# kristofbc/physical-interaction-video-prediction

Measured on AMD Instinct MI355X. Metric: predicted frames/sec (64x64x3, 10-step rollout), higher is better.
Workload: dtype f32; 1 GPU; CDNA rollout forward (Model.__call__, feed-self), batch 32/GPU, 10-frame 64x64x3 sequences, action-conditioned, num_masks=10, random-init weights; global_batch=32, parallelism=replicas x1

## Files before the change

### include/pivp_hip.h

```cpp
#ifndef PIVP_HIP_H
#define PIVP_HIP_H

#ifdef __cplusplus
extern "C" {
#endif

#define PIVP_OK 0
#define PIVP_ERR_BADARG (-1)
#define PIVP_ERR_LAUNCH (-2)
#define PIVP_ERR_STATE (-3)

#define PIVP_MODEL_CDNA 0
#define PIVP_MODEL_STP 1
#define PIVP_MODEL_DNA 2

#define PIVP_PRECISION_F32 0
#define PIVP_PRECISION_BF16 1
#define PIVP_PRECISION_BF16X3 2
#define PIVP_PRECISION_BF16X6 3
#define PIVP_PRECISION_FP16X3 4

int pivp_abi_version(void);

const char* pivp_build_digest(void);
const char* pivp_build_flags(void);

typedef struct pivp_plan pivp_plan_t;

typedef struct pivp_config {
    int batch;
    int seq_len;
    int height, width;
    int num_masks;
    int model_type;
    int use_state;
    int context_frames;
    int keep_activations;
    float ln_eps;
    int stp_zero_border;
    int action_dim;
    int state_dim;
} pivp_config_t;

int pivp_plan_create(const pivp_config_t* cfg, pivp_plan_t** out);
void pivp_plan_destroy(pivp_plan_t* plan);

int pivp_param_count(const pivp_plan_t* plan);
const char* pivp_param_name(const pivp_plan_t* plan, int idx);
long long pivp_param_numel(const pivp_plan_t* plan, int idx);
int pivp_plan_set_param(pivp_plan_t* plan, int idx, const float* dptr);

int pivp_plan_set_precision(pivp_plan_t* plan, int precision);
int pivp_plan_get_precision(const pivp_plan_t* plan);
int pivp_plan_set_deterministic(pivp_plan_t* plan, int on);
int pivp_plan_get_deterministic(const pivp_plan_t* plan);
enum { PIVP_OPT_SIDE_STREAM = 0, PIVP_OPT_FINISH_RIDER, PIVP_OPT_FUSE_ENC3, PIVP_OPT_LN_FOLD_TRAIN, PIVP_OPT_WGRAD_BATCH, PIVP_OPT_COUNT };
int pivp_plan_set_option(pivp_plan_t* plan, int option, int value);
int pivp_plan_get_option(const pivp_plan_t* plan, int option);
int pivp_plan_set_pack_cache(pivp_plan_t* plan, int on);
int pivp_plan_params_changed(pivp_plan_t* plan);

long long pivp_plan_workspace_bytes(const pivp_plan_t* plan);
int pivp_plan_set_workspace(pivp_plan_t* plan, void* dptr, long long bytes);

int pivp_reset_state(pivp_plan_t* plan, void* stream);

int pivp_rollout_forward(pivp_plan_t* plan, const float* images, const float* actions, const float* states,
                         const unsigned char* gt_select, float* gen_images, float* gen_states, float* results,
                         void* stream);

int pivp_rollout_predict(pivp_plan_t* plan, const float* context_images, const float* actions, const float* state0,
                         const float* track_in, int track_planes, int track_frame,
                         float* gen_images, float* gen_states, float* track_out, void* stream);

int pivp_plan_set_main_priority(pivp_plan_t* plan, int mode);

int pivp_plan_set_grad(pivp_plan_t* plan, int idx, float* dptr);
#define PIVP_GRAD_GROUPS 6
typedef void (*pivp_grad_group_cb)(void* user, int group);
int pivp_param_group(const pivp_plan_t* plan, int idx);
int pivp_param_group_by_name(const char* name);
int pivp_plan_set_grad_callback(pivp_plan_t* plan, pivp_grad_group_cb cb, void* user);
int pivp_plan_set_group_join(pivp_plan_t* plan, int join);
int pivp_plan_group_wait(pivp_plan_t* plan, int group, void* stream);
int pivp_rollout_backward(pivp_plan_t* plan, const float* images, const float* actions, const float* states,
                          const unsigned char* gt_select, const float* gen_images, const float* gen_states, void* stream);

int pivp_plan_set_profiling(pivp_plan_t* plan, int enable);
int pivp_plan_profile_read(pivp_plan_t* plan, double* ms_per_layer, int* launches_per_layer, double* flops_per_layer);

long long pivp_get_tap(pivp_plan_t* plan, const char* name, int step, float* out, void* stream);


int pivp_convlstm(const float* x, int cx, int ldx, const float* h_prev, int C, const float* w, const float* bias,
                  const float* c_in, float* c_out, float* h_out, int B, int H, int W, void* stream);

int pivp_convlstm_v(const float* x, int cx, int ldx, const float* h_prev, int C, const float* w, const float* bias,
                    const float* c_in, float* c_out, float* h_out, int B, int H, int W, int variant, void* stream);

long long pivp_convlstm_ln_scratch_floats(int B, int H, int W, int C);
int pivp_convlstm_ln(const float* x, int cx, int ldx, const float* h_prev, int C, const float* w, const float* bias,
                     const float* c_in, float* c_out, float* h_out, const float* gamma, const float* beta, float* ln_out,
                     int ldo, float* partials, float eps, int B, int H, int W, int variant, int* fused, void* stream);

long long pivp_lstm_bf16_weight_elems(int cin_total, int C);
int pivp_pack_lstm_bf16(const float* w, void* w_bf16, int cin_total, int C, void* stream);
int pivp_convlstm_bf16(const float* x, int cx, int ldx, const float* h_prev, int C, const void* w_bf16, const float* bias,
                       const float* c_in, float* c_out, float* h_out, float* gates_out, float* ln_part, int ln_cap,
                       int* ln_nparts, int B, int H, int W, int nch, void* stream);

int pivp_pack_lstm_bf16x3(const float* w, void* w_bf16, int cin_total, int C, void* stream);
int pivp_convlstm_bf16x3(const float* x, int cx, int ldx, const float* h_prev, int C, const void* w_bf16, const float* bias,
                         const float* c_in, float* c_out, float* h_out, float* gates_out, float* ln_part, int ln_cap,
                         int* ln_nparts, int B, int H, int W, int nch, void* stream);

int pivp_pack_lstm_bf16x6(const float* w, void* w_bf16, int cin_total, int C, void* stream);
int pivp_convlstm_bf16x6(const float* x, int cx, int ldx, const float* h_prev, int C, const void* w_bf16, const float* bias,
                         const float* c_in, float* c_out, float* h_out, float* gates_out, float* ln_part, int ln_cap,
                         int* ln_nparts, int B, int H, int W, int nch, void* stream);

int pivp_pack_lstm_fp16x3(const float* w, void* w_bf16, int cin_total, int C, int map_width, void* stream);
int pivp_convlstm_fp16x3(const float* x, int cx, int ldx, const float* h_prev, int C, const void* w_bf16, const float* bias,
                         const float* c_in, float* c_out, float* h_out, float* gates_out, float* ln_part, int ln_cap,
                         int* ln_nparts, int B, int H, int W, int nch, void* stream);

int pivp_deconv3x3s2_bf16(const float* x, int cin, int ldx, const float* w, const float* bias, float* out, int cout,
                          int ldo, int relu, int B, int Hin, int Win, void* stream);
int pivp_deconv3x3s2_bf16x3(const float* x, int cin, int ldx, const float* w, const float* bias, float* out, int cout,
                            int ldo, int relu, int B, int Hin, int Win, void* stream);
int pivp_deconv3x3s2_fp16x3(const float* x, int cin, int ldx, const float* w, const float* bias, float* out, int cout,
                            int ldo, int relu, int B, int Hin, int Win, float* scratch, void* stream);

long long pivp_conv5x5_bf16_weight_elems(int cin, int cout);
int pivp_conv5x5_bf16(const float* x, int cin, int ldx, const float* w, void* w_bf16, float* out, int cout, int ldo, int accum,
                      int B, int H, int W, void* stream);
int pivp_conv5x5_bf16x3(const float* x, int cin, int ldx, const float* w, void* w_bf16, float* out, int cout, int ldo, int accum,
                        int B, int H, int W, void* stream);
int pivp_conv5x5_bf16x6(const float* x, int cin, int ldx, const float* w, void* w_bf16, float* out, int cout, int ldo, int accum,
                        int B, int H, int W, void* stream);
int pivp_conv5x5_fp16x3(const float* x, int cin, int ldx, const float* w, void* w_bf16, float* out, int cout, int ldo, int accum,
                        int B, int H, int W, float* scratch, void* stream);
int pivp_conv5x5_ep(int precision, const float* x, int cin, int ldx, const float* w, void* w_bf16, float* out, int cout, int ldo, int accum,
                    const float* ep_src, int ep_ld, int ep_cols, int ep_mode, int no_split, float* scratch, int* applied,
                    int B, int H, int W, void* stream);
int pivp_conv5x5_ep_ksplit(int precision, int cin, int cout, int ldo, int accum, int no_split, int B, int H, int W);

int pivp_wgrad5x5_bf16(const float* x, int cx, int ldx, const float* h_prev, int C, const float* dG, float* dW, float* db,
                       int B, int H, int W, void* stream);
int pivp_wgrad5x5_bf16_batch(const float* x, int cx, int ldx, const float* h_prev, int C, const float* dG, float* dW, float* db,
                             int B, int H, int W, int tcount, long long ts_x, long long ts_h, long long ts_dG, void* stream);
int pivp_wgrad5x5_bf16_batch_form(const float* x, int cx, int ldx, const float* h_prev, int C, const float* dG, float* dW, float* db,
                                  int B, int H, int W, int tcount, long long ts_x, long long ts_h, long long ts_dG, int form, void* stream);
int pivp_wgrad5x5_bf16x6_batch(const float* x, int cx, int ldx, const float* h_prev, int C, const float* dG, float* dW, float* db,
                               int B, int H, int W, int tcount, long long ts_x, long long ts_h, long long ts_dG, void* stream);
int pivp_wgrad5x5_fp16x3_batch(const float* x, int cx, int ldx, const float* h_prev, int C, const float* dG, float* dW, float* db,
                               int B, int H, int W, int tcount, long long ts_x, long long ts_h, long long ts_dG, float* scratch, void* stream);

long long pivp_wgrad5x5_f32_part_floats(int cx, int C, int B, int H, int W, int form);
int pivp_wgrad5x5_f32_batch(const float* x, int cx, int ldx, const float* h_prev, int C, const float* dG, float* part, int overwrite,
                            float* dW, float* db, int B, int H, int W, int tcount, long long ts_x, long long ts_h, long long ts_dG, int form, void* stream);
int pivp_wgrad5x5_f32_reduce(int cx, int C, int has_h, float* part, float* dW, float* db, int B, int H, int W, int form, void* stream);
int pivp_wgrad5x5_f32_partition(int cx, int C, int has_h, int B, int H, int W, int form, int* geom8, int* segs, int seg_cap, int* nsegs,
                                int* slots, int slot_cap, int* nslots);
int pivp_conv5x5_f32(const float* x, int cin, int ldx, const float* wt, float* out, int cout, int B, int H, int W, void* stream);

int pivp_convlstm_train(const float* x, int cx, int ldx, const float* h_prev, int C, const float* w, const float* bias,
                        const float* c_in, float* c_out, float* h_out, float* gates_out, int B, int H, int W, void* stream);
int pivp_convlstm_backward(const float* x, int cx, int ldx, const float* h_prev, int C, const float* w, const float* gates,
                           const float* c_old, const float* c_new, const float* dh_a, int lda, const float* dh_b, int ldb,
                           float* dc, int dc_valid, float* dG, float* wt, float* d_in, float* dW, float* db,
                           int B, int H, int W, void* stream);
int pivp_conv_backward(int mode, const float* x, int cin, int ldx, const float* w, const float* dy, int cout, int ldy,
                       float* wt, float* dx, int lddx, int accum_dx, float* dW, float* db, int B, int Hin, int Win, void* stream);
long long pivp_conv_backward_part_floats(int mode, int cin, int cout, int B, int Hin, int Win);
int pivp_conv_wgrad_partial(int mode, const float* x, int cin, int ldx, const float* dy, int cout, int ldy, float* part,
                            float* dW, float* db, int B, int Hin, int Win, int repeats, void* stream);
int pivp_conv_wgrad_partial_batch(int mode, const float* x, int cin, int ldx, long long x_step_bytes, const float* dy, int cout, int ldy,
                                  long long dy_step_bytes, int tcount, int overwrite, float* part, float* dW, float* db, int B, int Hin, int Win,
                                  void* stream);
// ... 130 lines not shown
```

### physical-interaction-video-prediction_amd/csrc/igemm_f32.hip

```cpp
#include <stdlib.h>
#include <stdio.h>
#include <type_traits>

#include "lstm_gate_epilogue.h"

namespace pivp {

constexpr int IG_P = 36;

template <int WM, int NTB, int KG = 1>
constexpr int ig_lds_bytes() { return KG * 2 * (32 * WM + 32 * NTB) * IG_P * 4; }

#ifdef PIVP_F32_STAMPS
__device__ long long pivp_f32_stamps[2048 * 8];
#define F32_STAMP(i) do { if (threadIdx.x == 0 && blockIdx.x < 2048 && blockIdx.y == 0 && blockIdx.z == 0) { \
    pivp_f32_stamps[blockIdx.x * 4 + (i)] = (long long)wall_clock64(); pivp_f32_stamps[2048 * 4 + blockIdx.x * 4 + (i)] = (long long)clock64(); } } while (0)
#else
#define F32_STAMP(i)
#endif

template <int WM, int WN, int NTB, bool LSTM, int KG = 1>
__global__ __launch_bounds__(256 * KG, (KG == 1 && LSTM && WM < 4) ? 2 : 1) void igemm_f32_kernel(const IgemmDesc d) {
    F32_STAMP(0);
    PIVP_SET_MAIN_PRIO();
    static_assert(WM * WN == 4, "4 waves");
    static_assert(KG == 1 || (KG == 2 && LSTM), "the in-block K split serves the ConvLSTM tile only");
    static_assert(!LSTM || NTB == 4, "ConvLSTM blocks own 4 gates x 32 channels");
    constexpr int BM = 32 * WM;
    constexpr int BN = 32 * NTB;
    constexpr int CB = 8 * NTB;
    constexpr int CPW = LSTM ? CB / WN : 32 / WN;
    constexpr int GPT = 32 / CPW;
    constexpr int TPW = LSTM ? 4 / GPT : NTB / WN;
    extern __shared__ __attribute__((aligned(16))) float lds_all[];
    constexpr int A_FLOATS = BM * IG_P, B_FLOATS = BN * IG_P;
    const int gid = KG > 1 ? __builtin_amdgcn_readfirstlane((int)threadIdx.x >> 8) : 0;
    float* const lds = lds_all + gid * 2 * (A_FLOATS + B_FLOATS);

    const int tid = KG > 1 ? (int)threadIdx.x & 255 : (int)threadIdx.x;
    const int lane = tid & 63;
    const int wave = __builtin_amdgcn_readfirstlane(tid >> 6);
    const int wm = wave % WM, wn = wave / WM;
    const int phase = (int)gridDim.y - 1 - (int)blockIdx.y;
    const int n_nblk = LSTM ? (d.C / CB) : (d.N / BN);
    int lid = blockIdx.x;
    if ((gridDim.x & 7) == 0) lid = (blockIdx.x & 7) * (gridDim.x >> 3) + (blockIdx.x >> 3);
    const int n_mblk = d.n_mblk;
    const int nblk = pivp_fdiv(lid, d.fd_mb_mul, d.fd_mb_sh);
    const int mblk = lid - nblk * n_mblk;
    const int m0 = mblk * BM;
    const int cin = d.c0 + d.c1;
    const int ncc = cin >> 5;
    const int py = phase >> 1, px = phase & 1;
    const bool deconv = LSTM ? false : d.deconv != 0;
    const int ksz = LSTM ? 5 : d.ksize, pad = LSTM ? 2 : d.pad;
    const int nty_all = deconv ? 1 + py : ksz;
    const int ntx = deconv ? 1 + px : ksz;
    const int ksplit = LSTM ? 1 : (int)gridDim.z;
    const int nchunks_tot = nty_all * ntx * ncc;
    const int z_begin = ksplit > 1 ? (int)((unsigned)(nchunks_tot * (int)blockIdx.z) / (unsigned)ksplit) : 0;
    const int z_end = ksplit > 1 ? (int)((unsigned)(nchunks_tot * ((int)blockIdx.z + 1)) / (unsigned)ksplit) : nchunks_tot;
    const int nchunks_all = z_end - z_begin;
    const int nchunks = nchunks_all / KG;
    const int chunk0 = z_begin + gid * nchunks;
    const int HWg = d.Hg * d.Wg;

    constexpr int NA = (BM * 8 + 255) / 256;
    constexpr int NB = BN * 8 / 256;
    constexpr unsigned OOB = 0xC0000000u;
    const int cvec = tid & 7;
    const int prow = tid >> 3;
    const __amdgpu_buffer_rsrc_t rs0 = __builtin_amdgcn_make_buffer_rsrc(const_cast<float*>(d.x0), 0, d.bytes0, 0x00020000);
    const __amdgpu_buffer_rsrc_t rs1 = __builtin_amdgcn_make_buffer_rsrc(const_cast<float*>(d.c1 ? d.x1 : d.x0), 0, d.c1 ? d.bytes1 : d.bytes0, 0x00020000);
    const __amdgpu_buffer_rsrc_t rsw = __builtin_amdgcn_make_buffer_rsrc(const_cast<float*>(d.w), 0, d.bytesw, 0x00020000);
    int a_off0[NA], a_off1[NA];
    unsigned a_mask[NA];
    auto anchors = [&]() {
#pragma unroll
    for (int j = 0; j < NA; ++j) {
        const int m = m0 + prow + 32 * j;
        if (m < d.M && prow + 32 * j < BM) {
            const int b = pivp_fdiv(m, d.fd_hw_mul, d.fd_hw_sh);
            const int rem = m - b * HWg;
            const int ay = pivp_fdiv(rem, d.fd_w_mul, d.fd_w_sh);
            const int ax = rem - ay * d.Wg;
            const int iy0 = ay * d.in_step, ix0 = ax * d.in_step;
            const int pix = b * d.Hin * d.Win + iy0 * d.Win + ix0;
            a_off0[j] = (pix * d.ld0 + cvec * 4) * 4;
            a_off1[j] = (pix * d.ld1 + cvec * 4) * 4;
            unsigned colm = 0, m25 = 0;
            if (deconv) {
#pragma unroll
                for (int t = 0; t < 5; ++t) {
                    const int dxx = (px + 1 - (px ? 2 * t : 1)) >> 1;
                    if (t < ntx && (unsigned)(ix0 + dxx) < (unsigned)d.Win) colm |= 1u << t;
                }
#pragma unroll
                for (int t = 0; t < 5; ++t) {
                    const int dyy = (py + 1 - (py ? 2 * t : 1)) >> 1;
                    if (t < nty_all && (unsigned)(iy0 + dyy) < (unsigned)d.Hin) m25 |= colm << (5 * t);
                }
            } else {
                auto run = [](int lo, int hi) -> unsigned { return hi >= lo ? ((2u << hi) - 1u) & ~((1u << lo) - 1u) : 0u; };
                colm = run(max(pad - ix0, 0), min(d.Win - 1 + pad - ix0, ntx - 1));
                const int rlo = max(pad - iy0, 0), rhi = min(d.Hin - 1 + pad - iy0, nty_all - 1);
                const unsigned rows = rhi >= rlo ? 0x108421u & ((2u << (5 * rhi)) - 1u) & ~((1u << (5 * rlo)) - 1u) : 0u;
                m25 = colm * rows;
            }
            a_mask[j] = m25;
        } else {
            a_off0[j] = a_off1[j] = 0;
            a_mask[j] = 0;
        }
    }
    };
    int b_goff[NB];
#pragma unroll
    for (int j = 0; j < NB; ++j) {
        const int r = prow + 32 * j;
        const int col = LSTM ? (r / CB) * d.C + nblk * CB + (r % CB) : nblk * BN + r;
        b_goff[j] = (col * 32 + cvec * 4) * 4;
    }
    const int lds_wa = (prow * IG_P + cvec * 4);

    f32x4 ras[2][NA];
    f32x4 rbs[2][NB];

    int l_cc = 0, l_ty = 0, l_tx = 0;
    if (KG > 1 || ksplit > 1) {
        const int tap = pivp_fdiv(chunk0, d.fd_cc_mul, d.fd_cc_sh);
        l_cc = chunk0 - tap * ncc; l_ty = LSTM ? tap / 5 : tap / ntx; l_tx = tap - l_ty * ntx;
    }
    int s_delta = 0, s_ld = 0, s_wbase = 0;
    unsigned s_bit = 0;
    bool s_first = true;
    int t_dy = 0, t_dx = 0, t_wi = 0, t_cbase = 0;
    auto stage_a = [&]() {
        if (deconv) {
            const int ky = py ? 2 * l_ty : 1, kx = px ? 2 * l_tx : 1;
            t_dy = (py + 1 - ky) >> 1; t_dx = (px + 1 - kx) >> 1; t_wi = ky * 3 + kx;
        } else {
            t_dy = l_ty - pad; t_dx = l_tx - pad; t_wi = l_ty * ksz + l_tx;
        }
        s_bit = __builtin_amdgcn_readfirstlane(1u << (l_ty * 5 + l_tx));
        const int ch = l_cc << 5;
        s_first = ch < d.c0;
        s_ld = s_first ? d.ld0 : d.ld1;
        t_cbase = s_first ? ch : ch - d.c0;
    };
    auto stage_b = [&]() {
        s_delta = __builtin_amdgcn_readfirstlane(((t_dy * d.Win + t_dx) * s_ld + t_cbase) * 4);
    };
    auto stage_c = [&]() {
        s_wbase = __builtin_amdgcn_readfirstlane((t_wi * (d.wcin >> 5) + l_cc) * (d.wN ? d.wN : d.N) * 128);
        ++l_cc;
        const bool w0 = l_cc == ncc;
        l_cc = w0 ? 0 : l_cc;
        l_tx += w0 ? 1 : 0;
        const bool w1 = l_tx == ntx;
        l_tx = w1 ? 0 : l_tx;
        l_ty += w1 ? 1 : 0;
    };
    auto stage_begin = [&]() { stage_a(); stage_b(); stage_c(); };
    auto load_piece = [&](auto SET, auto J) {
        constexpr int j = decltype(J)::value;
        f32x4 (&ra)[NA] = ras[decltype(SET)::value];
        f32x4 (&rb)[NB] = rbs[decltype(SET)::value];
        if constexpr (j < NA) {
            const bool ok = (a_mask[j] & s_bit) != 0;
            unsigned off = ok ? (unsigned)((s_first ? a_off0[j] : a_off1[j]) + s_delta) : OOB;
            ra[j] = __builtin_bit_cast(f32x4, s_first ? __builtin_amdgcn_raw_buffer_load_b128(rs0, off, 0, 0)
                                                      : __builtin_amdgcn_raw_buffer_load_b128(rs1, off, 0, 0));
        } else if constexpr (j < NA + NB) {
            rb[j - NA] = __builtin_bit_cast(f32x4, __builtin_amdgcn_raw_buffer_load_b128(rsw, b_goff[j - NA], s_wbase, 0));
        }
    };
    auto store_piece = [&](auto SET, auto J, int buf) {
        constexpr int j = decltype(J)::value;
        const f32x4 (&ra)[NA] = ras[decltype(SET)::value];
        const f32x4 (&rb)[NB] = rbs[decltype(SET)::value];
        if constexpr (j < NA) {
            if (BM >= 32 * (j + 1)) *reinterpret_cast<f32x4*>(lds + buf * A_FLOATS + lds_wa + 32 * j * IG_P) = ra[j];
        } else if constexpr (j < NA + NB) {
            *reinterpret_cast<f32x4*>(lds + 2 * A_FLOATS + buf * B_FLOATS + lds_wa + 32 * (j - NA) * IG_P) = rb[j - NA];
        }
    };

    constexpr int NACC = LSTM ? (TPW == 1 ? 4 : TPW == 2 ? 2 : 1) : 1;
    f32x16 accs[NACC][TPW];
    f32x16 (&acc)[TPW] = accs[0];

    const int half = lane >> 5;
    const int l31 = lane & 31;
    const int a_off = (wm * 32 + l31) * IG_P + 4 * half;
    int b_off[TPW];
#pragma unroll
    for (int t = 0; t < TPW; ++t) {
        int row;
        if (LSTM) row = (t * GPT + l31 / CPW) * CB + wn * CPW + (l31 % CPW);
        else      row = (wn * TPW + t) * 32 + l31;
        b_off[t] = 2 * A_FLOATS + row * IG_P + 4 * half;
    }

    constexpr int NST = NA + NB;
    static_assert(NST <= 8, "staging pieces must fit the 16 micro-steps twice");
    constexpr int PRE = NST < 8 ? NST : 0;
    f32x4 fa[2];
    f32x4 fb[2][TPW];
    auto read_frag0 = [&](int slot) {
        fa[0] = *reinterpret_cast<const f32x4*>(lds + slot * A_FLOATS + a_off);
#pragma unroll
        for (int t = 0; t < TPW; ++t) fb[0][t] = *reinterpret_cast<const f32x4*>(lds + slot * B_FLOATS + b_off[t]);
    };
    auto chunk = [&](auto LOAD, auto STORE, auto SET, auto PAR, int buf) {
        constexpr bool do_load = decltype(LOAD)::value;
        constexpr bool do_store = decltype(STORE)::value;
        using OTHER = std::integral_constant<int, decltype(SET)::value ^ 1>;
        const float* As = lds + buf * A_FLOATS + a_off;
        const float* Bs = lds + buf * B_FLOATS;
        read_frag0(buf);
        __builtin_amdgcn_sched_barrier(0);
        auto micro = [&](auto Q, auto S2) {
            constexpr int q = decltype(Q)::value, s2 = decltype(S2)::value, step = q * 4 + s2;
            constexpr int cur = q & 1, nxt = cur ^ 1;
            constexpr int ci = NACC == 1 ? 0 : NACC == 2 ? decltype(PAR)::value : 2 * decltype(PAR)::value + (q & 1);
            if constexpr (s2 == 0 && q < 3) {
                fa[nxt] = *reinterpret_cast<const f32x4*>(As + 8 * (q + 1));
#pragma unroll
                for (int t = 0; t < TPW; ++t) fb[nxt][t] = *reinterpret_cast<const f32x4*>(Bs + b_off[t] + 8 * (q + 1));
            }
#pragma unroll
            for (int t = 0; t < TPW; ++t)
                accs[ci][t] = __builtin_amdgcn_mfma_f32_32x32x2f32(fa[cur][s2], fb[cur][t][s2], accs[ci][t], 0, 0, 0);
            if constexpr (do_load && PRE == 0 && step == 0) stage_begin();
            if constexpr (do_load && PRE > 0 && step == PRE) stage_a();
            if constexpr (do_load && PRE > 0 && step == PRE + 1) stage_b();
            if constexpr (do_load && PRE > 0 && step == PRE + 2) stage_c();
            if constexpr (do_load && step < NST) load_piece(SET, std::integral_constant<int, step>{});
            if constexpr (do_store && step >= 16 - NST) store_piece(OTHER{}, std::integral_constant<int, step - (16 - NST)>{}, buf ^ 1);
            __builtin_amdgcn_sched_barrier(0);
        };
        auto qgroup = [&](auto Q) {
            micro(Q, std::integral_constant<int, 0>{}); micro(Q, std::integral_constant<int, 1>{});
            micro(Q, std::integral_constant<int, 2>{}); micro(Q, std::integral_constant<int, 3>{});
        };
        qgroup(std::integral_constant<int, 0>{}); qgroup(std::integral_constant<int, 1>{});
        qgroup(std::integral_constant<int, 2>{}); qgroup(std::integral_constant<int, 3>{});
    };
    using S0 = std::integral_constant<int, 0>; using S1 = std::integral_constant<int, 1>;
    auto load_all = [&](auto SET) {
        load_piece(SET, std::integral_constant<int, 0>{}); load_piece(SET, std::integral_constant<int, 1>{});
        load_piece(SET, std::integral_constant<int, 2>{}); load_piece(SET, std::integral_constant<int, 3>{});
        load_piece(SET, std::integral_constant<int, 4>{}); load_piece(SET, std::integral_constant<int, 5>{});
        load_piece(SET, std::integral_constant<int, 6>{}); load_piece(SET, std::integral_constant<int, 7>{});
    };
    auto store_all = [&](auto SET, int buf) {
        store_piece(SET, std::integral_constant<int, 0>{}, buf); store_piece(SET, std::integral_constant<int, 1>{}, buf);
        store_piece(SET, std::integral_constant<int, 2>{}, buf); store_piece(SET, std::integral_constant<int, 3>{}, buf);
        store_piece(SET, std::integral_constant<int, 4>{}, buf); store_piece(SET, std::integral_constant<int, 5>{}, buf);
        store_piece(SET, std::integral_constant<int, 6>{}, buf); store_piece(SET, std::integral_constant<int, 7>{}, buf);
    };
    auto sync = [&]() { __syncthreads(); };
    auto load_b = [&](auto SET) {
        if constexpr (NB > 0) load_piece(SET, std::integral_constant<int, NA + 0>{});
        if constexpr (NB > 1) load_piece(SET, std::integral_constant<int, NA + 1>{});
        if constexpr (NB > 2) load_piece(SET, std::integral_constant<int, NA + 2>{});
        if constexpr (NB > 3) load_piece(SET, std::integral_constant<int, NA + 3>{});
    };
    auto load_a = [&](auto SET) {
        if constexpr (NA > 0) load_piece(SET, std::integral_constant<int, 0>{});
        if constexpr (NA > 1) load_piece(SET, std::integral_constant<int, 1>{});
        if constexpr (NA > 2) load_piece(SET, std::integral_constant<int, 2>{});
        if constexpr (NA > 3) load_piece(SET, std::integral_constant<int, 3>{});
    };
    static_assert(NA <= 4 && NB <= 4, "load_a / load_b unroll four pieces each");

    if (nchunks > 0) { stage_begin(); load_b(S0{}); }
    __builtin_amdgcn_sched_barrier(0);
    anchors();
    if (nchunks > 0) load_a(S0{});
    __builtin_amdgcn_sched_barrier(0);

    constexpr int OWNR = LSTM ? 16 / GPT : 1;
    float cpre[OWNR];
    float bj = 0.f, bi = 0.f, bf = 0.f, bo = 0.f;
    if constexpr (LSTM) {
        const int C = d.C, ch = nblk * CB + wn * CPW + (l31 % CPW), grp = l31 / CPW;
        bj = d.bias[ch]; bi = d.bias[C + ch]; bf = d.bias[2 * C + ch] + 1.0f; bo = d.bias[3 * C + ch];
        const __amdgpu_buffer_rsrc_t rsci = __builtin_amdgcn_make_buffer_rsrc(const_cast<float*>(d.cstate_in), 0, d.M * C * 4, 0x00020000);
        const int voc = ((m0 + wm * 32 + 4 * half + (GPT > 1 ? grp : 0)) * C + ch) * 4;
#pragma unroll
        for (int k = 0; k < OWNR; ++k) {
            const int srow = GPT == 1 ? (k & 3) + 8 * (k >> 2) : GPT == 2 ? 2 * (k & 1) + 8 * (k >> 1) : 8 * k;
            cpre[k] = __builtin_bit_cast(float, __builtin_amdgcn_raw_buffer_load_b32(rsci, voc, srow * C * 4, 0));
        }
    }

#pragma unroll
    for (int a = 0; a < NACC; ++a)
#pragma unroll
        for (int n = 0; n < TPW; ++n)
#pragma unroll
            for (int r = 0; r < 16; ++r) accs[a][n][r] = 0.f;
    if (nchunks > 0) {
        store_all(S0{}, 0);
        if (nchunks > 1) { stage_begin(); load_all(S1{}); }
        if constexpr (PRE > 0) stage_begin();
        __syncthreads();
        F32_STAMP(1);
        int it = 0;
        for (; it + 3 < nchunks; it += 2) {
            chunk(std::true_type{}, std::true_type{}, S0{}, S0{}, 0); sync();
            chunk(std::true_type{}, std::true_type{}, S1{}, S1{}, 1); sync();
        }
        const int rest = nchunks - it;
        if (rest == 3) {
            chunk(std::true_type{}, std::true_type{}, S0{}, S0{}, 0); sync();
            chunk(std::false_type{}, std::true_type{}, S1{}, S1{}, 1); sync();
            chunk(std::false_type{}, std::false_type{}, S0{}, S0{}, 0);
        } else if (rest == 2) {
            chunk(std::false_type{}, std::true_type{}, S0{}, S0{}, 0); sync();
            chunk(std::false_type{}, std::false_type{}, S0{}, S1{}, 1);
        } else {
            chunk(std::false_type{}, std::false_type{}, S0{}, S0{}, 0);
        }
    }
    F32_STAMP(2);
    if constexpr (NACC > 1) {
#pragma unroll
        for (int t = 0; t < TPW; ++t)
#pragma unroll
            for (int r = 0; r < 16; ++r) {
                if constexpr (NACC == 2) accs[0][t][r] = accs[0][t][r] + accs[1][t][r];
                else accs[0][t][r] = (accs[0][t][r] + accs[1][t][r]) + (accs[2][t][r] + accs[3][t][r]);
            }
    }

    if constexpr (KG > 1) {
        __syncthreads();
        float* xch = lds_all;
        if (gid == 1) {
#pragma unroll
            for (int t = 0; t < TPW; ++t)
#pragma unroll
                for (int r = 0; r < 16; ++r) xch[(t * 16 + r) * 256 + tid] = accs[0][t][r];
        }
        __syncthreads();
        if (gid == 1) {
            if (LSTM && d.ln_part) { __syncthreads(); __syncthreads(); __syncthreads(); }
            return;
        }
#pragma unroll
        for (int t = 0; t < TPW; ++t)
#pragma unroll
            for (int r = 0; r < 16; ++r) accs[0][t][r] += xch[(t * 16 + r) * 256 + tid];
    }

    auto tile_stats = [&](const float* v, auto ownmask, auto NV, int b, int slot) {
        constexpr int nv = decltype(NV)::value;
        float s1 = 0.f, c1 = 0.f;
#pragma unroll
        for (int i = 0; i < nv; ++i)
            if ((ownmask >> i) & 1) { s1 += v[i]; c1 += 1.f; }
        s1 = wave_sum(s1); c1 = wave_sum(c1);
        __syncthreads();
        if (lane == 0) { lds[wave] = s1; lds[4 + wave] = c1; }
        __syncthreads();
        const float cnt = (lds[4] + lds[5]) + (lds[6] + lds[7]);
        const float mean = ((lds[0] + lds[1]) + (lds[2] + lds[3])) / cnt;
        float q = 0.f;
#pragma unroll
        for (int i = 0; i < nv; ++i)
            if ((ownmask >> i) & 1) { const float dd = v[i] - mean; q = fmaf(dd, dd, q); }
        q = wave_sum(q);
        if (lane == 0) lds[8 + wave] = q;
        __syncthreads();
        if (tid == 0) {
            float* p = d.ln_part + ((size_t)b * d.ln_nparts + slot) * 4;
            p[0] = cnt; p[1] = mean; p[2] = (lds[8] + lds[9]) + (lds[10] + lds[11]); p[3] = 0.f;
        }
    };
    if constexpr (LSTM) {
        const int C = d.C;
        const int ch = nblk * CB + wn * CPW + (l31 % CPW);
        const int grp = l31 / CPW;
        const int M = d.M;
        const __amdgpu_buffer_rsrc_t rsc = __builtin_amdgcn_make_buffer_rsrc(d.cstate_out, 0, M * C * 4, 0x00020000);
        const __amdgpu_buffer_rsrc_t rsh = __builtin_amdgcn_make_buffer_rsrc(d.hout, 0, M * C * 4, 0x00020000);
        const __amdgpu_buffer_rsrc_t rsg = __builtin_amdgcn_make_buffer_rsrc(d.gates_out ? d.gates_out : d.hout, 0, d.gates_out ? M * C * 16 : 0, 0x00020000);
        const int mlane = m0 + wm * 32 + 4 * half + (GPT > 1 ? grp : 0);
        const int vo = (mlane * C + ch) * 4, vog = (mlane * 4 * C + ch) * 4;
        float sv[OWNR];
        unsigned own = 0;
#pragma unroll
        for (int k = 0; k < OWNR; ++k) {
            float g4[4];
#pragma unroll
            for (int t = 0; t < 4 / GPT; ++t) {
                float rows[GPT], got[GPT];
#pragma unroll
                for (int g = 0; g < GPT; ++g) rows[g] = acc[t][k * GPT + g];
                gate_exchange<GPT, CPW>(rows, grp, got);
#pragma unroll
                for (int g = 0; g < GPT; ++g) g4[t * GPT + g] = got[g];
            }
            const int srow = GPT == 1 ? (k & 3) + 8 * (k >> 2) : GPT == 2 ? 2 * (k & 1) + 8 * (k >> 1) : 8 * k;
            const int so = srow * C * 4;
            const LstmCell cell = lstm_cell<GateActF32>(g4, bj, bi, bf, bo, cpre[k]);
            __builtin_amdgcn_raw_buffer_store_b32(__builtin_bit_cast(unsigned, cell.c), rsc, vo, so, 0);
            __builtin_amdgcn_raw_buffer_store_b32(__builtin_bit_cast(unsigned, cell.h), rsh, vo, so, 0);
            const bool in = mlane + srow < M;
            sv[k] = in ? cell.h : 0.f;
            own |= in ? 1u << k : 0u;
            if (d.gates_out) {
                const int sog = so * 4;
                __builtin_amdgcn_raw_buffer_store_b32(__builtin_bit_cast(unsigned, cell.aj), rsg, vog, sog, 0);
                __builtin_amdgcn_raw_buffer_store_b32(__builtin_bit_cast(unsigned, cell.ai), rsg, vog, sog + C * 4, 0);
                __builtin_amdgcn_raw_buffer_store_b32(__builtin_bit_cast(unsigned, cell.af), rsg, vog, sog + C * 8, 0);
                __builtin_amdgcn_raw_buffer_store_b32(__builtin_bit_cast(unsigned, cell.ao), rsg, vog, sog + C * 12, 0);
            }
        }
        if (d.ln_part) {
            const int b = pivp_fdiv(m0, d.fd_hw_mul, d.fd_hw_sh);
            tile_stats(sv, own, std::integral_constant<int, OWNR>{}, b, ((m0 - b * HWg) / BM) * n_nblk + nblk);
        }
    } else if (!deconv && d.out_step == 1 && d.Hout == d.Hg && d.Wout == d.Wg && !d.bias && !d.relu && !d.accum && !d.ln_part &&
               (long long)d.M * d.ldo * 4 < (1LL << 31)) {
        const __amdgpu_buffer_rsrc_t rso = __builtin_amdgcn_make_buffer_rsrc(d.out, 0, d.M * d.ldo * 4, 0x00020000);
        const int vo = ((m0 + wm * 32 + 4 * half) * d.ldo + nblk * BN + wn * TPW * 32 + l31) * 4;
        const int row4 = __builtin_amdgcn_readfirstlane(d.ldo * 4);
        if (ksplit > 1) {
            if (nchunks > 0) {
#pragma unroll
                for (int r = 0; r < 16; ++r)
#pragma unroll
                    for (int t = 0; t < TPW; ++t)
                        __builtin_amdgcn_raw_ptr_buffer_atomic_fadd_f32(acc[t][r], rso, vo + t * 128, ((r & 3) + 8 * (r >> 2)) * row4, 0);
            }
        } else {
#pragma unroll
            for (int r = 0; r < 16; ++r)
#pragma unroll
                for (int t = 0; t < TPW; ++t) {
                    const float v = acc[t][r];
                    __builtin_amdgcn_raw_buffer_store_b32(__builtin_bit_cast(unsigned, v), rso, vo + t * 128, ((r & 3) + 8 * (r >> 2)) * row4, 0);
                }
        }
    } else {
        const int oy0 = deconv ? py : 0, ox0 = deconv ? px : 0;
        float sv[16 * TPW];
        unsigned long long own = 0;
#pragma unroll
        for (int r = 0; r < 16; ++r) {
            const int m = m0 + wm * 32 + (r & 3) + 8 * (r >> 2) + 4 * half;
            if (m < d.M) {
                const int b = pivp_fdiv(m, d.fd_hw_mul, d.fd_hw_sh);
                const int rem = m - b * HWg;
                const int ay = pivp_fdiv(rem, d.fd_w_mul, d.fd_w_sh);
                const int ax = rem - ay * d.Wg;
                const int opix = (ay * d.out_step + oy0) * d.Wout + ax * d.out_step + ox0;
                const size_t o = ((size_t)b * d.Hout * d.Wout + opix) * d.ldo;
#pragma unroll
                for (int t = 0; t < TPW; ++t) {
                    const int col = nblk * BN + (wn * TPW + t) * 32 + l31;
                    if (ksplit > 1) {
                        if (nchunks > 0) atomicAdd(d.out + o + col, acc[t][r]);
                    } else {
                        float v = acc[t][r] + (d.bias ? d.bias[col] : 0.f);
                        if (d.relu) v = fmaxf(v, 0.f);
                        if (d.accum) v += d.out[o + col];
                        d.out[o + col] = v;
                        sv[t * 16 + r] = v; own |= 1ull << (t * 16 + r);
                    }
                }
            }
        }
        if (d.ln_part) {
            const int b = pivp_fdiv(m0, d.fd_hw_mul, d.fd_hw_sh);
            tile_stats(sv, own, std::integral_constant<int, 16 * TPW>{}, b,
                       (((m0 - b * HWg) / BM) * n_nblk + nblk) * (int)gridDim.y + phase);
        }
    }
#ifdef PIVP_F32_STAMPS
    asm volatile("s_waitcnt vmcnt(0)" ::: "memory");
    F32_STAMP(3);
#endif
}

template <int WM, int WN, int NTB, bool LSTM, int KG = 1>
static int launch_igemm(const IgemmDesc& d, hipStream_t stream, int ksplit = 1, int* ln_nparts = nullptr) {
    constexpr int BM = 32 * WM, BN = 32 * NTB;
    const int n_nblk = LSTM ? (d.C / (8 * NTB)) : (d.N / BN);
    const int mblk = (d.M + BM - 1) / BM;
    constexpr int lds_bytes = ig_lds_bytes<WM, NTB, KG>();
    static PerDeviceOnce once;
    if (pivp_ensure_dyn_lds(once, reinterpret_cast<const void*>(&igemm_f32_kernel<WM, WN, NTB, LSTM, KG>), lds_bytes) != PIVP_OK) return PIVP_ERR_LAUNCH;
    dim3 grid(mblk * n_nblk, d.nphase, ksplit);
    IgemmDesc dd = d;
    dd.n_mblk = mblk;
    pivp_fastdiv((unsigned)mblk, &dd.fd_mb_mul, &dd.fd_mb_sh);
    pivp_fastdiv((unsigned)(d.Hg * d.Wg), &dd.fd_hw_mul, &dd.fd_hw_sh);
    pivp_fastdiv((unsigned)d.Wg, &dd.fd_w_mul, &dd.fd_w_sh);
    pivp_fastdiv((unsigned)((d.c0 + d.c1) >> 5), &dd.fd_cc_mul, &dd.fd_cc_sh);
    const int hwg = d.Hg * d.Wg;
    const int np = (hwg / BM) * n_nblk * d.nphase;
    dd.ln_nparts = (d.ln_part && ksplit == 1 && hwg % BM == 0 && np <= d.ln_cap) ? np : 0;
    if (!dd.ln_nparts) dd.ln_part = nullptr;
    if (ln_nparts) *ln_nparts = dd.ln_nparts;
    hipLaunchKernelGGL((igemm_f32_kernel<WM, WN, NTB, LSTM, KG>), grid, dim3(256 * KG), lds_bytes, stream, dd);
    return PIVP_LAUNCH_STATUS();
}

int igemm_validate(const IgemmDesc& d, bool lstm) {
    PIVP_CHECK_ARG(d.x0 && d.w && d.c0 > 0 && d.c0 % 32 == 0 && d.c1 % 32 == 0 && d.c1 >= 0);
    PIVP_CHECK_ARG(d.c1 == 0 || d.x1);
    PIVP_CHECK_ARG(d.ld0 >= d.c0 && d.ld0 % 4 == 0 && (d.c1 == 0 || (d.ld1 >= d.c1 && d.ld1 % 4 == 0)));
    PIVP_CHECK_ARG(d.B > 0 && d.Hin > 0 && d.Win > 0 && d.Hg > 0 && d.Wg > 0 && d.in_step >= 1);
    PIVP_CHECK_ARG(d.M == d.B * d.Hg * d.Wg);
    PIVP_CHECK_ARG(d.deconv ? (d.nphase == 4 && d.in_step == 1 && d.out_step == 2) : (d.nphase == 1 && d.ksize >= 1 && d.ksize <= 5 && d.pad >= 0));
    PIVP_CHECK_ARG(d.bytes0 > 0 && d.bytesw > 0 && (d.c1 == 0 || d.bytes1 > 0));
    PIVP_CHECK_ARG(d.wcin >= d.c0 + d.c1 && d.wcin % 32 == 0);
    if (lstm) {
        PIVP_CHECK_ARG(d.C > 0 && d.C % 32 == 0 && d.N == 4 * d.C && d.bias && d.cstate_in && d.cstate_out && d.hout);
        PIVP_CHECK_ARG(d.nphase == 1 && d.in_step == 1 && d.Hg == d.Hin && d.Wg == d.Win && d.ksize == 5 && d.pad == 2 && !d.deconv);
        PIVP_CHECK_ARG((long long)d.M * d.C * 4 < (1LL << 31));
    } else {
        PIVP_CHECK_ARG(d.out && d.N % 32 == 0 && d.N >= 32 && d.ldo >= d.N);
        PIVP_CHECK_ARG(d.out_step >= 1 && d.Hout > 0 && d.Wout > 0);
        PIVP_CHECK_ARG((d.Hg - 1) * d.out_step + (d.deconv ? 1 : 0) < d.Hout && (d.Wg - 1) * d.out_step + (d.deconv ? 1 : 0) < d.Wout);
    }
    return PIVP_OK;
}

int igemm_lstm(const IgemmDesc& d, hipStream_t stream, int variant, int* ln_nparts) {
    int rc = igemm_validate(d, true);
    if (rc != PIVP_OK) return rc;
    if (variant == 0) {
        const long nb = d.C / 32;
        if ((long)(d.M / 64) * nb >= 512) variant = 2;
        else if ((long)(d.M / 64) * nb >= 256) variant = 4;
        else variant = 3;
    }
    switch (variant) {
        case 4:
            if (((25 * ((d.c0 + d.c1) >> 5)) & 1) == 0) return launch_igemm<2, 2, 4, true, 2>(d, stream, 1, ln_nparts);
            return launch_igemm<2, 2, 4, true>(d, stream, 1, ln_nparts);
        case 1: return launch_igemm<4, 1, 4, true>(d, stream, 1, ln_nparts);
        case 2: return launch_igemm<2, 2, 4, true>(d, stream, 1, ln_nparts);
        case 3: {
            const int ncc = (d.c0 + d.c1) >> 5;
            if (((25 * ncc) & 1) == 0) return launch_igemm<1, 4, 4, true, 2>(d, stream, 1, ln_nparts);
            return launch_igemm<1, 4, 4, true>(d, stream, 1, ln_nparts);
        }
    }
    return PIVP_ERR_BADARG;
}

static bool dgrad_choice(const IgemmDesc& d, int& bt, int& bks) {
    if (!((d.ksplit_ok || d.no_ksplit) && !d.deconv && !d.bias && !d.relu && !d.accum && d.ksize * d.ksize * ((d.c0 + d.c1) / 32) > 40)) return false;
    const int ks_max = d.no_ksplit ? 1 : 10;
    const int nt = d.N / 32;
    struct Tile { int wm, wn, ntb; double eff; int resident; };
    static const Tile tiles[] = {{2, 2, 2, 0.80, 4}, {4, 1, 1, 0.70, 3}, {4, 1, 2, 0.90, 2}, {4, 1, 3, 0.95, 2}, {4, 1, 4, 1.00, 1}, {2, 2, 4, 0.95, 2}, {1, 4, 4, 0.80, 3}};
    static const double fixed_taps[] = {3.0, 1.5, 1.0, 1.0};
    static const double alone[] = {0.90, 1.0, 1.0, 1.0};
    const int cus = pivp_cu_count();
    bt = -1; bks = 1;
    double bcost = 1e300;
    const int nchunks = d.ksize * d.ksize * ((d.c0 + d.c1) / 32);
    const double split_penalty = 1.01 + 0.14 * (d.M >= 32768 ? 1.0 : d.M / 32768.0);
    for (int t = 0; t < 7; ++t) {
        if (nt % tiles[t].ntb) continue;
        const int bm = 32 * tiles[t].wm, bn = 32 * tiles[t].ntb;
        const long mb = (d.M + bm - 1) / bm, nb = d.N / bn;
        for (int ks = 1; ks <= ks_max && ks * 8 <= nchunks; ++ks) {
            const long blocks = mb * nb * ks;
            const long per_cu = (blocks + cus - 1) / cus;
            const int res = (int)(per_cu < tiles[t].resident ? per_cu : tiles[t].resident);
            const double taps = (double)(d.ksize * d.ksize) / ks;
            const double cost = (double)per_cu * bm * bn * (taps + fixed_taps[res - 1]) / (tiles[t].eff * alone[res - 1]) * (ks > 1 ? split_penalty : 1.0);
            if (cost < bcost) { bcost = cost; bt = t; bks = ks; }
        }
    }
    return bt >= 0;
}
int igemm_conv_ksplit(const IgemmDesc& d) {
    int bt, bks;
    return dgrad_choice(d, bt, bks) ? bks : 1;
}

int igemm_conv(const IgemmDesc& d, hipStream_t stream, int* ln_nparts) {
    int rc = igemm_validate(d, false);
    if (rc != PIVP_OK) return rc;
    int bt = -1, bks = 1;
    const bool dgrad = dgrad_choice(d, bt, bks);
    const bool aligned = d.ldo % 4 == 0 && ((uintptr_t)d.out & 15) == 0 && (!d.bias || ((uintptr_t)d.bias & 15) == 0);
    const bool tile_ok = deconv_tile_ok(d);
    switch (conv_form(d.deconv, d.c0 + d.c1, d.N, d.B, tile_ok ? d.Hin : 1, d.Win, aligned, dgrad, d.ksize, d.M)) {
        case ConvForm::DeconvTile: return deconv_tile(d, stream, ln_nparts);
        case ConvForm::LongKDgrad:
            switch (bt) {
                case 0: return launch_igemm<2, 2, 2, false>(d, stream, bks, ln_nparts);
                case 1: return launch_igemm<4, 1, 1, false>(d, stream, bks, ln_nparts);
                case 2: return launch_igemm<4, 1, 2, false>(d, stream, bks, ln_nparts);
                case 3: return launch_igemm<4, 1, 3, false>(d, stream, bks, ln_nparts);
                case 4: return launch_igemm<4, 1, 4, false>(d, stream, bks, ln_nparts);
                case 5: return launch_igemm<2, 2, 4, false>(d, stream, bks, ln_nparts);
                case 6: return launch_igemm<1, 4, 4, false>(d, stream, bks, ln_nparts);
            }
            return PIVP_ERR_BADARG;
        case ConvForm::Small1: case ConvForm::Small2: case ConvForm::Small3: return igemm_small(d, stream, ln_nparts);
        case ConvForm::F32_128x32: return launch_igemm<4, 1, 1, false>(d, stream, 1, ln_nparts);
        case ConvForm::F32_128x64: return launch_igemm<4, 1, 2, false>(d, stream, 1, ln_nparts);
        case ConvForm::F32_128x96: return launch_igemm<4, 1, 3, false>(d, stream, 1, ln_nparts);
        case ConvForm::F32_128x128: return launch_igemm<4, 1, 4, false>(d, stream, 1, ln_nparts);
        case ConvForm::F32_64x64: return launch_igemm<2, 2, 2, false>(d, stream, 1, ln_nparts);
        case ConvForm::F32_64x128: return launch_igemm<2, 2, 4, false>(d, stream, 1, ln_nparts);
        case ConvForm::F32_32x128: return launch_igemm<1, 4, 4, false>(d, stream, 1, ln_nparts);
    }
    return PIVP_ERR_BADARG;
}

}

#ifdef PIVP_F32_STAMPS
extern "C" int pivp_debug_f32_stamps(long long* out, int n) {
    return hipMemcpyFromSymbol(out, HIP_SYMBOL(pivp::pivp_f32_stamps), sizeof(long long) * n) == hipSuccess ? 0 : -2;
}
#endif

PIVP_DEFINE_MAIN_PRIO_SETTER(igemm_f32)
// ... 1 lines not shown
```

### physical-interaction-video-prediction_amd/csrc/pivp_c_api.hip

```cpp
#include <string.h>
#include <string>
#include <vector>

#include "../../include/pivp_hip.h"
#include "../../include/pivp_data.h"
#include "../../include/pivp_conv_forms.h"
#include "pivp_host.h"

using namespace pivp;

namespace pivp {

long long view_bytes(int B, int H, int W, int ld) { return (long long)B * H * W * ld * 4; }
bool fits31(long long v) { return v > 0 && v < (1LL << 31); }
int run_convlstm(const float* x, int cx, int ldx, const float* h_prev, int C, const float* w, const float* bias,
                 const float* c_in, float* c_out, float* h_out, int B, int H, int W, hipStream_t s, const ConvLstmOpts& o) {
    const LnIn* const ln_in = o.ln_in;
    const bool l2d = operand_l2_direct(o.operand);
    if ((o.w_bf16 != nullptr) != (o.operand != Operand::F32)) return PIVP_ERR_BADARG;
    IgemmDesc d;
    memset(&d, 0, sizeof(d));
    if (ln_in) {
        if (!convlstm_ln_in_ok(o.operand, cx, ldx, C, B, H, W) || !ln_in->gamma || !ln_in->beta || !ln_in->part || ln_in->np <= 0 || ln_in->part == o.ln_out.part)
            return PIVP_ERR_BADARG;
        d.in_g = ln_in->gamma; d.in_b = ln_in->beta; d.in_part = ln_in->part; d.in_np = ln_in->np; d.in_eps = ln_in->eps;
    }
    d.x0 = x; d.c0 = cx; d.ld0 = ldx; d.x1 = h_prev; d.c1 = h_prev ? C : 0; d.ld1 = C; d.wcin = cx + C;
    d.w = w; d.bias = bias;
    d.B = B; d.Hin = H; d.Win = W; d.Hg = H; d.Wg = W; d.in_step = 1;
    d.N = 4 * C; d.M = B * H * W;
    d.nphase = 1; d.deconv = 0; d.ksize = 5; d.pad = 2;
    const long long b0 = view_bytes(B, H, W, ldx), b1 = view_bytes(B, H, W, C), bw = 25LL * (cx + C) * 4 * C * 4;
    if (!fits31(b0) || !fits31(b1) || !fits31(bw) || (o.gates_out && !fits31(4 * b1))) return PIVP_ERR_BADARG;
    d.bytes0 = (int)b0; d.bytes1 = (int)b1; d.bytesw = (int)bw;
    d.out_step = 1; d.Hout = H; d.Wout = W;
    d.cstate_in = c_in; d.cstate_out = c_out; d.hout = h_out; d.C = C; d.gates_out = o.gates_out;
    d.ln_part = o.ln_out.part; d.ln_cap = o.ln_out.cap;
    if (l2d && !convlstm_bf16_ok(d)) return w ? igemm_lstm(d, s, 0, o.ln_out.nparts) : PIVP_ERR_BADARG;
    if (o.w_bf16) return convlstm_bf16(d, o.w_bf16, s, o.operand, o.ln_out.nparts, (l2d && o.variant != 16 && o.variant != 32) ? 0 : o.variant);
    return igemm_lstm(d, s, o.variant, o.ln_out.nparts);
}

bool convlstm_ln_in_ok(Operand form, int cx, int ldx, int C, int B, int H, int W) {
    return operand_l2_direct(form) && cx <= 64 && ldx == cx && cx % 8 == 0 && C % 16 == 0 && H % 8 == 0 && W % 16 == 0;
}
static int conv3x3s2_desc(IgemmDesc& d, const float* x, int cin, int ldx, const float* w, const float* bias, float* out, int cout,
                          int ldo, int relu, int B, int Hin, int Win, int accum) {
    if (Hin % 2 || Win % 2) return PIVP_ERR_BADARG;
    memset(&d, 0, sizeof(d));
    d.x0 = x; d.c0 = cin; d.ld0 = ldx; d.wcin = cin; d.w = w; d.bias = bias;
    d.B = B; d.Hin = Hin; d.Win = Win; d.Hg = Hin / 2; d.Wg = Win / 2; d.in_step = 2;
    d.N = cout; d.M = B * d.Hg * d.Wg;
    d.nphase = 1; d.deconv = 0; d.ksize = 3; d.pad = 1;
    const long long b0 = view_bytes(B, Hin, Win, ldx), bw = 9LL * cin * cout * 4;
    if (!fits31(b0) || !fits31(bw)) return PIVP_ERR_BADARG;
    d.bytes0 = (int)b0; d.bytesw = (int)bw;
    d.out_step = 1; d.Hout = d.Hg; d.Wout = d.Wg; d.out = out; d.ldo = ldo; d.relu = relu; d.accum = accum;
    return PIVP_OK;
}
int run_conv3x3s2(const float* x, int cin, int ldx, const float* w, const float* bias, float* out, int cout,
                  int ldo, int relu, int B, int Hin, int Win, hipStream_t s, int accum) {
    IgemmDesc d;
    int rc = conv3x3s2_desc(d, x, cin, ldx, w, bias, out, cout, ldo, relu, B, Hin, Win, accum);
    if (rc != PIVP_OK) return rc;
    return igemm_conv(d, s);
}

static void conv3x3s2_ln_desc(IgemmDesc& d, const float* x_raw, int cin, const float* w, const float* bias, float* out, int cout, int ldo,
                              int relu, int B, int Hin, int Win) {
    memset(&d, 0, sizeof(d));
    d.x0 = x_raw; d.c0 = cin; d.ld0 = cin; d.wcin = cin; d.w = w; d.bias = bias;
    d.B = B; d.Hin = Hin; d.Win = Win; d.Hg = Hin / 2; d.Wg = Win / 2; d.in_step = 2;
    d.N = cout; d.M = B * d.Hg * d.Wg;
    d.nphase = 1; d.deconv = 0; d.ksize = 3; d.pad = 1;
    d.out_step = 1; d.Hout = d.Hg; d.Wout = d.Wg; d.out = out; d.ldo = ldo; d.relu = relu;
}
bool conv3x3s2_ln_ok(int cin, int cout, int B, int Hin, int Win) {
    if (Hin % 2 || Win % 2 || cin % 32 || cout % 32) return false;
    IgemmDesc d;
    conv3x3s2_ln_desc(d, nullptr, cin, nullptr, nullptr, nullptr, cout, cout, 0, B, Hin, Win);
    return igemm_in_ln_ok(d) && fits31(view_bytes(B, Hin, Win, cin)) && fits31(9LL * cin * cout * 4);
}
int run_conv3x3s2_ln(const float* x_raw, int cin, const float* w, const float* bias, float* out, int cout, int ldo, int relu,
                     int B, int Hin, int Win, hipStream_t s, const LnIn& ln, const Conv3x3LnOpts& o) {
    if (!x_raw || !w || !out || !ln.gamma || !ln.beta || !ln.part || ln.np <= 0 || !conv3x3s2_ln_ok(cin, cout, B, Hin, Win)) return PIVP_ERR_BADARG;
    IgemmDesc d;
    conv3x3s2_ln_desc(d, x_raw, cin, w, bias, out, cout, ldo, relu, B, Hin, Win);
    d.bytes0 = (int)view_bytes(B, Hin, Win, cin); d.bytesw = (int)(9LL * cin * cout * 4);
    d.in_g = ln.gamma; d.in_b = ln.beta; d.in_part = ln.part; d.in_np = ln.np; d.in_eps = ln.eps;
    d.in_out = o.keep.out; d.in_out_ld = o.keep.ld; d.in_stat_out = o.keep.stat;
    if (o.fuse3 && o.fuse3->e3) {
        if (cout != 64 || ldo != 64 || !relu || !bias) return PIVP_ERR_BADARG;
        d.f3_w = o.fuse3->w3; d.f3_b = o.fuse3->b3; d.f3_action = o.fuse3->action; d.f3_state = o.fuse3->state; d.f3_wcs = o.fuse3->wcs; d.f3_bcs = o.fuse3->bcs;
        d.f3_out = o.fuse3->e3; d.f3_state_out = o.fuse3->state_out; d.f3_use_state = o.fuse3->use_state;
    }
    int rc = igemm_validate(d, false);
    if (rc != PIVP_OK) return rc;
    return igemm_small(d, s);
}

static int deconv3x3s2_desc(IgemmDesc& d, const float* x0, int c0, int ld0, const float* x1, int c1, int ld1, const float* w, const float* bias,
                            float* out, int cout, int ldo, int relu, int B, int Hin, int Win) {
    memset(&d, 0, sizeof(d));
    d.x0 = x0; d.c0 = c0; d.ld0 = ld0; d.x1 = x1; d.c1 = x1 ? c1 : 0; d.ld1 = ld1; d.wcin = c0 + d.c1; d.w = w; d.bias = bias;
    d.B = B; d.Hin = Hin; d.Win = Win; d.Hg = Hin; d.Wg = Win; d.in_step = 1;
    d.N = cout; d.M = B * Hin * Win;
    d.nphase = 4; d.deconv = 1; d.ksize = 3; d.pad = 1;
    const long long b0 = view_bytes(B, Hin, Win, ld0), b1 = d.c1 ? view_bytes(B, Hin, Win, ld1) : 0, bw = 9LL * d.wcin * cout * 4;
    if (!fits31(b0) || (d.c1 && !fits31(b1)) || !fits31(bw)) return PIVP_ERR_BADARG;
    d.bytes0 = (int)b0; d.bytes1 = (int)b1; d.bytesw = (int)bw;
    d.out_step = 2; d.Hout = 2 * Hin; d.Wout = 2 * Win; d.out = out; d.ldo = ldo; d.relu = relu;
    return PIVP_OK;
}
static bool deconv_form_ok(Operand form, const float* wscale_part) { return form != Operand::BF16X6 && (!operand_needs_scale(form) || wscale_part); }
int run_deconv3x3s2(const float* x, int cin, int ldx, const float* w, const float* bias, float* out, int cout,
                    int ldo, int relu, int B, int Hin, int Win, hipStream_t s, const DeconvOpts& o) {
    if (!deconv_form_ok(o.operand, o.wscale_part)) return PIVP_ERR_BADARG;
    IgemmDesc d;
    int rc = deconv3x3s2_desc(d, x, cin, ldx, nullptr, 0, 0, w, bias, out, cout, ldo, relu, B, Hin, Win);
// ... 222 lines not shown
    if (rc != PIVP_OK) return rc;
    return fork_end(a.fork);
}

int run_layernorm(const float* x, const float* g, const float* b, float* out, float* partials, int B, int n, int C,
                  int ldo, float eps, int relu, hipStream_t s, const LayerNormOpts& o) {
    if (o.fused_nparts <= 0) {
        int rc = ln_stats(x, partials, B, n, s);
        if (rc != PIVP_OK) return rc;
    }
    return ln_apply(x, partials, g, b, out, B, n, C, ldo, eps, relu, s, o.stat_out, o.fused_nparts);
}

__global__ __launch_bounds__(256) void select_frames_kernel(const float* __restrict__ gt, const float* __restrict__ gen,
                                                            const unsigned char* __restrict__ take, float* __restrict__ out,
                                                            int frame_numel) {
    const int b = blockIdx.y;
    const float* src = take[b] ? gt : gen;
    const size_t base = (size_t)b * frame_numel;
    for (int i = (blockIdx.x * 256 + threadIdx.x) * 4; i < frame_numel; i += gridDim.x * 1024)
        *reinterpret_cast<f32x4*>(out + base + i) = *reinterpret_cast<const f32x4*>(src + base + i);
}

int run_select_frames(const float* gt, const float* gen, const unsigned char* take, float* out, int B, int frame_numel, hipStream_t s) {
    if (!gt || !gen || !take || !out || B <= 0 || frame_numel <= 0 || frame_numel % 4) return PIVP_ERR_BADARG;
    hipLaunchKernelGGL(select_frames_kernel, dim3(8, B), dim3(256), 0, s, gt, gen, take, out, frame_numel);
    return PIVP_LAUNCH_STATUS();
}

int run_conv_backward(const ConvBwdArgs& a, hipStream_t s) {
    const int mode = a.mode, B = a.B, Hin = a.Hin, Win = a.Win;
    const int Hout = mode ? 2 * Hin : Hin / 2, Wout = mode ? 2 * Win : Win / 2;
    int rc = PIVP_OK;
    if (a.y) { rc = relu_mask(a.dy, a.ldy, a.y, a.ldyy, a.cout, (long)B * Hout * Wout, s, a.dy_add, a.ld_add); if (rc != PIVP_OK) return rc; }
    else if (a.dy_add) { rc = add_strided(a.dy, a.ldy, a.dy_add, a.ld_add, a.cout, (long)B * Hout * Wout, s); if (rc != PIVP_OK) return rc; }
    hipStream_t sw;
    rc = fork_begin(a.fork, s, &sw);
    if (rc != PIVP_OK) return rc;
    if (a.dx) {
        if (!a.wt_ready) {
            rc = repack_transpose(a.w, a.wt, 9, a.cin, a.cout, 0, s);
            if (rc != PIVP_OK) return rc;
        }
        DeconvOpts o{};
        o.accum = a.accum_dx; o.operand = a.operand;
        rc = mode ? run_conv3x3s2(a.dy, a.cout, a.ldy, a.wt, nullptr, a.dx, a.cin, a.lddx, 0, B, Hout, Wout, s, a.accum_dx)
                  : run_deconv3x3s2(a.dy, a.cout, a.ldy, a.wt, nullptr, a.dx, a.cin, a.lddx, 0, B, Hout, Wout, s, o);
        if (rc != PIVP_OK) return rc;
    }
    if (!a.dW) return PIVP_OK;
    WgradDesc d;
    conv3x3s2_wgrad_geom(d, mode, a.cin, a.cout, B, Hin, Win);
    d.x0 = a.x; d.ld0 = a.ldx; d.dy = a.dy; d.ldy = a.ldy; d.dw = a.dW; d.db = a.db; d.part = a.part;
    rc = run_wgrad(d, sw, Operand::F32);
    if (rc != PIVP_OK) return rc;
    return fork_end(a.fork);
}

}

#ifndef PIVP_BUILD_DIGEST
#define PIVP_BUILD_DIGEST "unstamped"
#endif
extern "C" const char* pivp_build_digest(void) { return PIVP_BUILD_DIGEST; }
#ifndef PIVP_BUILD_FLAGS
#define PIVP_BUILD_FLAGS ""
#endif
extern "C" const char* pivp_build_flags(void) { return PIVP_BUILD_FLAGS; }
extern "C" int pivp_abi_version(void) { return 17; }

static bool ep_args_ok(const float* ep_src, int ep_ld, int ep_cols, int ep_mode, int cout) {
    if (ep_mode < 0 || ep_mode > 2) return false;
    if (!ep_src || !ep_mode) return true;
    return ep_ld >= (ep_cols < cout ? ep_cols : cout);
}
static bool form_serves_map(Operand form, int B, int H, int W) { return form == Operand::F32 || packed_tiles_serve(H, W, B); }
extern "C" int pivp_convlstm(const float* x, int cx, int ldx, const float* h_prev, int C, const float* w, const float* bias,
                             const float* c_in, float* c_out, float* h_out, int B, int H, int W, void* stream) {
    if (!x || !w || !bias || !c_in || !c_out || !h_out) return PIVP_ERR_BADARG;
    return run_convlstm(x, cx, ldx, h_prev, C, w, bias, c_in, c_out, h_out, B, H, W, (hipStream_t)stream);
}
extern "C" int pivp_convlstm_v(const float* x, int cx, int ldx, const float* h_prev, int C, const float* w, const float* bias,
                               const float* c_in, float* c_out, float* h_out, int B, int H, int W, int variant, void* stream) {
    if (!x || !w || !bias || !c_in || !c_out || !h_out || variant < 0 || variant > 4) return PIVP_ERR_BADARG;
    ConvLstmOpts o{};
    o.variant = variant;
    return run_convlstm(x, cx, ldx, h_prev, C, w, bias, c_in, c_out, h_out, B, H, W, (hipStream_t)stream, o);
}
extern "C" int pivp_convlstm_train(const float* x, int cx, int ldx, const float* h_prev, int C, const float* w, const float* bias,
                                   const float* c_in, float* c_out, float* h_out, float* gates_out, int B, int H, int W, void* stream) {
    if (!x || !w || !bias || !c_in || !c_out || !h_out || !gates_out) return PIVP_ERR_BADARG;
    ConvLstmOpts o{};
    o.gates_out = gates_out;
    return run_convlstm(x, cx, ldx, h_prev, C, w, bias, c_in, c_out, h_out, B, H, W, (hipStream_t)stream, o);
}
static int convlstm_backward_op(const float* x, int cx, int ldx, const float* h_prev, int C, const float* w, const float* gates,
                                const float* c_old, const float* c_new, const float* dh_a, int lda, const float* dh_b, int ldb,
                                float* dc, int dc_valid, float* dG, float* wt, float* d_in, float* dW, float* db,
                                int B, int H, int W, void* stream, int dx_only) {
    if (!x || !w || !gates || !c_old || !c_new || !dc || !dG || !wt || !d_in || !dW || !db) return PIVP_ERR_BADARG;
    ConvLstmBwdArgs a{};
    a.x = x; a.cx = cx; a.ldx = ldx; a.h_prev = h_prev; a.C = C; a.w = w; a.gates = gates; a.c_old = c_old; a.c_new = c_new;
    a.dh_a = dh_a; a.lda = lda; a.dh_b = dh_b; a.ldb = ldb; a.dc = dc; a.dc_valid = dc_valid; a.dG = dG; a.wt = wt; a.d_in = d_in;
    a.dW = dW; a.db = db; a.B = B; a.H = H; a.W = W;
    a.dx_only = dx_only;
    return run_convlstm_backward(a, (hipStream_t)stream);
}
extern "C" int pivp_convlstm_backward(const float* x, int cx, int ldx, const float* h_prev, int C, const float* w, const float* gates,
                                      const float* c_old, const float* c_new, const float* dh_a, int lda, const float* dh_b, int ldb,
                                      float* dc, int dc_valid, float* dG, float* wt, float* d_in, float* dW, float* db,
                                      int B, int H, int W, void* stream) {
    return convlstm_backward_op(x, cx, ldx, h_prev, C, w, gates, c_old, c_new, dh_a, lda, dh_b, ldb, dc, dc_valid, dG, wt, d_in, dW, db, B, H, W, stream, 0);
}
extern "C" int pivp_conv_backward(int mode, const float* x, int cin, int ldx, const float* w, const float* dy, int cout, int ldy,
                                  float* wt, float* dx, int lddx, int accum_dx, float* dW, float* db, int B, int Hin, int Win,
                                  void* stream) {
    if (!x || !w || !dy || !wt || !dW || !db || mode < 0 || mode > 1) return PIVP_ERR_BADARG;
    ConvBwdArgs a{};
    a.mode = mode; a.x = x; a.cin = cin; a.ldx = ldx; a.w = w; a.dy = const_cast<float*>(dy); a.cout = cout; a.ldy = ldy;
    a.wt = wt; a.dx = dx; a.lddx = lddx; a.accum_dx = accum_dx; a.dW = dW; a.db = db; a.B = B; a.Hin = Hin; a.Win = Win;
    return run_conv_backward(a, (hipStream_t)stream);
}
extern "C" long long pivp_conv_backward_part_floats(int mode, int cin, int cout, int B, int Hin, int Win) {
    if (mode < 0 || mode > 1 || cin <= 0 || cout <= 0 || B <= 0 || Hin <= 0 || Win <= 0) return PIVP_ERR_BADARG;
    return conv_backward_part_floats(mode, cin, cout, B, Hin, Win);
}
extern "C" int pivp_conv_wgrad_partial(int mode, const float* x, int cin, int ldx, const float* dy, int cout, int ldy, float* part,
                                       float* dW, float* db, int B, int Hin, int Win, int repeats, void* stream) {
    if (!x || !dy || !part || !dW || !db || mode < 0 || mode > 1 || repeats < 1) return PIVP_ERR_BADARG;
    WgradDesc desc;
    conv3x3s2_wgrad_geom(desc, mode, cin, cout, B, Hin, Win);
    desc.x0 = x; desc.ld0 = ldx; desc.dy = dy; desc.ldy = ldy; desc.dw = dW; desc.db = db; desc.part = part;
    for (int r = 0; r < repeats; ++r) {
        const int rc = run_wgrad(desc, (hipStream_t)stream, Operand::F32);
        if (rc != PIVP_OK) return rc;
    }
    return igemm_wgrad_reduce(desc, (hipStream_t)stream);
}
extern "C" int pivp_conv_wgrad_partial_batch(int mode, const float* x, int cin, int ldx, long long x_step_bytes, const float* dy, int cout, int ldy,
                                             long long dy_step_bytes, int tcount, int overwrite, float* part, float* dW, float* db, int B, int Hin, int Win,
                                             void* stream) {
    if (!x || !dy || !part || !dW || !db || mode < 0 || mode > 1 || tcount < 1) return PIVP_ERR_BADARG;
    WgradDesc d;
    conv3x3s2_wgrad_geom(d, mode, cin, cout, B, Hin, Win);
    d.x0 = x; d.ld0 = ldx; d.dy = dy; d.ldy = ldy; d.dw = dW; d.db = db;
    d.tcount = tcount; d.ts_x0 = x_step_bytes; d.ts_dy = dy_step_bytes;
    d.part = part; d.part_overwrite = overwrite ? 1 : 0;
    return run_wgrad(d, (hipStream_t)stream, Operand::F32);
}
extern "C" int pivp_conv_wgrad_partial_reduce(int mode, int cin, int cout, float* part, float* dW, float* db, int B, int Hin, int Win, void* stream) {
    if (!part || !dW || !db || mode < 0 || mode > 1) return PIVP_ERR_BADARG;
    WgradDesc d;
    conv3x3s2_wgrad_geom(d, mode, cin, cout, B, Hin, Win);
    d.part = part; d.dw = dW; d.db = db;
    return igemm_wgrad_reduce(d, (hipStream_t)stream);
}
static void lstm_wgrad_op(WgradDesc& d, const float* x, int cx, int ldx, const float* h_prev, int C, const float* dG, float* dW, float* db,
                          int B, int H, int W, int tcount, long long ts_x, long long ts_h, long long ts_dG) {
    lstm_wgrad_geom(d, cx, C, B, H, W);
    d.x0 = x; d.ld0 = ldx; d.x1 = h_prev; d.dy = dG; d.dw = dW; d.db = db;
    d.tcount = tcount; d.ts_x0 = ts_x; d.ts_x1 = ts_h; d.ts_dy = ts_dG;
}
extern "C" long long pivp_wgrad5x5_f32_part_floats(int cx, int C, int B, int H, int W, int form) {
    if (cx <= 0 || C <= 0 || B <= 0 || H <= 0 || W <= 0 || form < 0 || form > 2) return PIVP_ERR_BADARG;
    return lstm_wgrad_part_floats(cx, C, B, H, W, form, 0);
}
extern "C" int pivp_wgrad5x5_f32_batch(const float* x, int cx, int ldx, const float* h_prev, int C, const float* dG, float* part, int overwrite,
                                       float* dW, float* db, int B, int H, int W, int tcount, long long ts_x, long long ts_h, long long ts_dG, int form,
                                       void* stream) {
// ... 160 lines not shown
    o.operand = Operand::FP16X3; o.ascale_part = scratch;
    return run_conv5x5_bf16(x, cin, ldx, (const unsigned short*)w_bf16, out, cout, ldo, accum, B, H, W, (hipStream_t)stream, o);
}
extern "C" int pivp_conv5x5_ep(int precision, const float* x, int cin, int ldx, const float* w, void* w_bf16, float* out, int cout, int ldo, int accum,
                               const float* ep_src, int ep_ld, int ep_cols, int ep_mode, int no_split, float* scratch, int* applied,
                               int B, int H, int W, void* stream) {
    if (applied) *applied = 0;
    if (precision < 1 || precision > 4 || !x || !w || !w_bf16 || !out || cin <= 0 || cout <= 0 || B <= 0 || H <= 0 || W <= 0) return PIVP_ERR_BADARG;
    const Operand form = (Operand)precision;
    if (!form_serves_map(form, B, H, W) || (operand_needs_scale(form) && (!scratch || ldx != cin)) || !ep_args_ok(ep_src, ep_ld, ep_cols, ep_mode, cout))
        return PIVP_ERR_BADARG;
    int rc = pack_lstm_bf16(w, (unsigned short*)w_bf16, cin, cout, (hipStream_t)stream, form, conv5x5_bf16_rows(cout), operand_l2_direct(form) ? 1 : 0);
    if (rc != PIVP_OK) return rc;
    if (operand_needs_scale(form)) {
        rc = absmax_partials(x, (long)B * H * W * cin, scratch, (hipStream_t)stream);
        if (rc != PIVP_OK) return rc;
    }
    const EpSpec ep{ep_src, ep_ld, ep_cols, ep_mode, applied};
    Conv5x5Bf16Opts o{};
    o.operand = form; o.no_split = no_split ? 1 : 0;
    if (operand_needs_scale(form)) o.ascale_part = scratch;
    if (ep_src && ep_mode) o.ep = &ep;
    return run_conv5x5_bf16(x, cin, ldx, (const unsigned short*)w_bf16, out, cout, ldo, accum, B, H, W, (hipStream_t)stream, o);
}
extern "C" int pivp_conv5x5_ep_ksplit(int precision, int cin, int cout, int ldo, int accum, int no_split, int B, int H, int W) {
    if (precision < 1 || precision > 4 || cin <= 0 || cout <= 0 || ldo < cout || B <= 0 || H <= 0 || W <= 0) return PIVP_ERR_BADARG;
    IgemmDesc d;
    static float dummy;
    if (conv5x5_bf16_desc(d, &dummy, cin, cin, &dummy, cout, ldo, accum, B, H, W) != PIVP_OK) return PIVP_ERR_BADARG;
    if (no_split) d.ksplit_ok = 0;
    return conv5x5_bf16_ksplit(d, (Operand)precision);
}
static int lstm_wgrad_packed_op(Operand operand, const float* x, int cx, int ldx, const float* h_prev, int C, const float* dG, float* dW, float* db, int B, int H,
                                int W, int tcount, long long ts_x, long long ts_h, long long ts_dG, int form, const float* dy_absmax, void* stream) {
    WgradDesc d;
    lstm_wgrad_op(d, x, cx, ldx, h_prev, C, dG, dW, db, B, H, W, tcount, ts_x, ts_h, ts_dG);
    d.form = form;
    if (dy_absmax) { d.dy_absmax = dy_absmax; d.dy_absmax_stride = 72; }
    return run_wgrad(d, (hipStream_t)stream, operand);
}
extern "C" int pivp_wgrad5x5_bf16(const float* x, int cx, int ldx, const float* h_prev, int C, const float* dG, float* dW, float* db,
                                  int B, int H, int W, void* stream) {
    if (!x || !dG || !dW || C <= 0 || cx <= 0) return PIVP_ERR_BADARG;
    return lstm_wgrad_packed_op(Operand::BF16, x, cx, ldx, h_prev, C, dG, dW, db, B, H, W, 1, 0, 0, 0, 0, nullptr, stream);
}
extern "C" int pivp_wgrad5x5_fp16x3_batch(const float* x, int cx, int ldx, const float* h_prev, int C, const float* dG, float* dW, float* db,
                                          int B, int H, int W, int tcount, long long ts_x, long long ts_h, long long ts_dG, float* scratch, void* stream) {
    if (!x || !dG || !dW || !scratch || C <= 0 || cx <= 0 || tcount < 1 || B <= 0 || H <= 0 || W <= 0) return PIVP_ERR_BADARG;
    if (!form_serves_map(Operand::FP16X3, B, H, W)) return PIVP_ERR_BADARG;
    for (int j = 0; j < tcount; ++j) {
        const int rc = absmax_partials(reinterpret_cast<const float*>(reinterpret_cast<const char*>(dG) + j * ts_dG), (long)B * H * W * 4 * C,
                                       scratch + (size_t)j * 72, (hipStream_t)stream);
        if (rc != PIVP_OK) return rc;
    }
    return lstm_wgrad_packed_op(Operand::FP16X3, x, cx, ldx, h_prev, C, dG, dW, db, B, H, W, tcount, ts_x, ts_h, ts_dG, 0, scratch, stream);
}
extern "C" int pivp_wgrad5x5_bf16x6_batch(const float* x, int cx, int ldx, const float* h_prev, int C, const float* dG, float* dW, float* db,
                                          int B, int H, int W, int tcount, long long ts_x, long long ts_h, long long ts_dG, void* stream) {
    if (!x || !dG || !dW || C <= 0 || cx <= 0 || tcount < 1) return PIVP_ERR_BADARG;
    return lstm_wgrad_packed_op(Operand::BF16X6, x, cx, ldx, h_prev, C, dG, dW, db, B, H, W, tcount, ts_x, ts_h, ts_dG, 0, nullptr, stream);
}
extern "C" int pivp_wgrad5x5_bf16_batch(const float* x, int cx, int ldx, const float* h_prev, int C, const float* dG, float* dW, float* db,
                                        int B, int H, int W, int tcount, long long ts_x, long long ts_h, long long ts_dG, void* stream) {
    if (!x || !dG || !dW || C <= 0 || cx <= 0 || tcount < 1) return PIVP_ERR_BADARG;
    return lstm_wgrad_packed_op(Operand::BF16, x, cx, ldx, h_prev, C, dG, dW, db, B, H, W, tcount, ts_x, ts_h, ts_dG, 0, nullptr, stream);
}
extern "C" int pivp_wgrad5x5_bf16_batch_form(const float* x, int cx, int ldx, const float* h_prev, int C, const float* dG, float* dW, float* db,
                                             int B, int H, int W, int tcount, long long ts_x, long long ts_h, long long ts_dG, int form, void* stream) {
    if (!x || !dG || !dW || C <= 0 || cx <= 0 || tcount < 1 || form < 0 || form > 2) return PIVP_ERR_BADARG;
    return lstm_wgrad_packed_op(Operand::BF16, x, cx, ldx, h_prev, C, dG, dW, db, B, H, W, tcount, ts_x, ts_h, ts_dG, form, nullptr, stream);
}
static int convlstm_ln_cap(int H, int W, int C) {
    const int tiles = ((H * W + 31) / 32) * (C / 32), slices = ln_stats_slices(H * W * C);
    return tiles > slices ? tiles : slices;
}
extern "C" long long pivp_convlstm_ln_scratch_floats(int B, int H, int W, int C) {
    if (B <= 0 || H <= 0 || W <= 0 || C <= 0 || C % 32) return PIVP_ERR_BADARG;
    return (long long)B * convlstm_ln_cap(H, W, C) * 4;
}
extern "C" int pivp_convlstm_ln(const float* x, int cx, int ldx, const float* h_prev, int C, const float* w, const float* bias,
                                const float* c_in, float* c_out, float* h_out, const float* gamma, const float* beta,
                                float* ln_out, int ldo, float* partials, float eps, int B, int H, int W, int variant, int* fused,
                                void* stream) {
    if (!x || !w || !bias || !c_in || !c_out || !h_out || !gamma || !beta || !ln_out || !partials || variant < 0 || variant > 4)
        return PIVP_ERR_BADARG;
    if (C <= 0 || C % 32) return PIVP_ERR_BADARG;
    int np = 0;
    ConvLstmOpts o{};
    o.variant = variant; o.ln_out.part = partials; o.ln_out.cap = convlstm_ln_cap(H, W, C); o.ln_out.nparts = &np;
    int rc = run_convlstm(x, cx, ldx, h_prev, C, w, bias, c_in, c_out, h_out, B, H, W, (hipStream_t)stream, o);
    if (rc != PIVP_OK) return rc;
    if (fused) *fused = np > 0;
    LayerNormOpts lo{};
    lo.fused_nparts = np;
    return run_layernorm(h_out, gamma, beta, ln_out, partials, B, H * W * C, C, ldo, eps, 0, (hipStream_t)stream, lo);
}
extern "C" long long pivp_layernorm_backward_scratch_floats(int B, int n) {
    if (B <= 0 || n <= 0) return PIVP_ERR_BADARG;
    return (long long)B * ln_bwd_slices(n) * 2;
}
extern "C" int pivp_layernorm_backward(const float* dy, int lddy, const float* y, int ldy, const float* x, const float* stat,
                                       const float* gamma, float* partials, float* dx, float* dgamma, float* dbeta,
                                       int B, int n, int C, int relu, void* stream) {
    return ln_backward(dy, lddy, y, ldy, x, stat, gamma, partials, dx, dgamma, dbeta, B, n, C, relu, (hipStream_t)stream);
}
extern "C" long long pivp_gates_backward_ln_scratch_floats(int B, int n) {
    if (B <= 0 || n <= 0) return PIVP_ERR_BADARG;
    return (long long)B * ln_bwd_slices(n) * 2 + ln_bwd_param_part_floats(n);
}
extern "C" int pivp_gates_backward_ln(const float* gates, const float* c_old, const float* c_new, const float* dy, int lddy,
                                      const float* gamma, const float* stat, const float* h, const float* dh_b, int ldb, float* dc,
                                      int dc_valid, float* dG, float* dgamma, float* dbeta, float* scratch, int B, int npix, int C,
                                      void* stream) {
    if (!gates || !c_old || !c_new || !dy || !gamma || !stat || !h || !dc || !dG || !dgamma || !dbeta || !scratch) return PIVP_ERR_BADARG;
    if (B <= 0 || npix <= 0 || C <= 0 || C % 4 || lddy < C || lddy % 4) return PIVP_ERR_BADARG;
    hipStream_t s = (hipStream_t)stream;
    const int n = npix * C;
    float* partials = scratch;
    float* part = scratch + (size_t)B * ln_bwd_slices(n) * 2;
    if (hipMemsetAsync(part, 0, (size_t)ln_bwd_param_part_floats(n) * 4, s) != hipSuccess) return PIVP_ERR_LAUNCH;
    LnFuse lf;
    memset(&lf, 0, sizeof(lf));
    lf.dy = dy; lf.lddy = lddy; lf.gamma = gamma; lf.stat = stat; lf.h = h;
    lf.partials = partials; lf.S = ln_bwd_slices(n);
    int rc = ln_backward(dy, lddy, nullptr, 0, h, stat, gamma, partials, nullptr, dgamma, dbeta, B, n, C, 0, s, part);
    if (rc != PIVP_OK) return rc;
    rc = lstm_gates_bwd(gates, c_old, c_new, nullptr, 0, dh_b, ldb, dc, dc_valid, dG, B * npix, C, s, B, &lf);
    if (rc != PIVP_OK) return rc;
    return ln_bwd_params_reduce(part, dgamma, dbeta, B, n, s);
}
extern "C" int pivp_composite_backward_tiles(int H, int W) {
    if (H <= 0 || W <= 0) return PIVP_ERR_BADARG;
    return composite_bwd_tiles(H, W);
}
extern "C" int pivp_composite_backward(int model_type, const float* prev, const float* mask_logits, const float* layer0, const float* aux,
                                       const float* go, float* dmk, float* dz, float* part, float* dprev, int dprev_accum, int B, int H, int W,
                                       int num_masks, int stp_zero_border, unsigned long long* det_acc, void* stream) {
    hipStream_t s = (hipStream_t)stream;
    if (model_type == PIVP_MODEL_CDNA) {
        if (det_acc) return PIVP_ERR_BADARG;
        return composite_bwd_cdna(prev, mask_logits, layer0, aux, go, dmk, dz, part, dprev, dprev_accum, B, H, W, num_masks, s);
    }
    if (model_type == PIVP_MODEL_STP) {
        if (dprev && !dprev_accum) return PIVP_ERR_BADARG;
        return composite_bwd_stp(prev, mask_logits, layer0, aux, go, dmk, dz, part, dprev, B, H, W, num_masks, stp_zero_border, s, det_acc);
    }
    if (model_type == PIVP_MODEL_DNA) {
        if (det_acc || num_masks != 1) return PIVP_ERR_BADARG;
        return composite_bwd_dna(prev, mask_logits, aux, go, dmk, dz, dprev, dprev_accum, B, H, W, s);
    }
    return PIVP_ERR_BADARG;
}
extern "C" int pivp_mask_softmax_backward(const float* mask_logits, float* dmk, int B, int HW, int NP, void* stream) {
    return mask_softmax_bwd(mask_logits, dmk, B, HW, NP, (hipStream_t)stream);
}
extern "C" long long pivp_heads_backward_det_floats(int B, int HW, int NP, int NE) {
    if (B <= 0 || HW <= 0 || NP <= 0 || NE <= 0) return PIVP_ERR_BADARG;
    return heads_bwd_det_floats(B, HW, NP, NE);
}
extern "C" int pivp_heads_backward(const float* e6, const float* wm, const float* we, const float* dpm, const float* dpe, float* de6,
                                   float* dwm, float* dbm, float* dwe, float* dbe, int B, int HW, int NP, int NE, float* det_part,
                                   void* stream) {
    if (NP <= 0 || NE <= 0) return PIVP_ERR_BADARG;
    return heads_bwd(e6, wm, we, dpm, dpe, de6, dwm, dbm, dwe, dbe, B, HW, NP, NE, (hipStream_t)stream, det_part);
}
extern "C" int pivp_cdna_kernels_backward(const float* hidden5, const float* wt, const float* vpre, const float* dkpart, int ntiles, float* dv,
                                          float* dhidden5, int accum_dx, float* dwt, float* db, int B, int K, int num_masks, float* det_part,
                                          void* stream) {
    if (ntiles <= 0) return PIVP_ERR_BADARG;
    return cdna_kernels_bwd(hidden5, wt, vpre, dkpart, ntiles, dv, dhidden5, accum_dx, dwt, db, B, K, num_masks, (hipStream_t)stream, nullptr, det_part);
}
extern "C" int pivp_stp_params_backward(const float* hidden5, const float* wt1, const float* s1, const float* w2, const float* dthpart, int ntiles,
// ... 273 lines not shown
```

### physical-interaction-video-prediction_amd/csrc/pivp_host.h

```cpp
#pragma once
#include "pivp_kernels.h"
#include "side_lane.h"
#include "sweep_schedule.h"

namespace pivp {

long long view_bytes(int B, int H, int W, int ld);
bool fits31(long long v);

struct LnIn { const float* gamma; const float* beta; const float* part; int np; float eps; };
struct LnPartOut { float* part; int cap; int* nparts; };
struct NormKeep { float* out; int ld; float* stat; };
struct Enc3Fuse { const float* w3; const float* b3; const float* action; const float* state; const float* wcs; const float* bcs; float* e3; float* state_out; int use_state; };
struct MotionRider { int mode, KS, nout; const float* partials; const float* bias; const float* w2; const float* b2; float* out; float* vpre; };
struct EpSpec { const float* src; int ld, cols, mode; int* applied; };

struct ConvLstmOpts {
    int variant;
    float* gates_out;
    LnPartOut ln_out;
    Operand operand;
    const unsigned short* w_bf16;
    const LnIn* ln_in;
};
bool convlstm_ln_in_ok(Operand form, int cx, int ldx, int C, int B, int H, int W);
int run_convlstm(const float* x, int cx, int ldx, const float* h_prev, int C, const float* w, const float* bias,
                 const float* c_in, float* c_out, float* h_out, int B, int H, int W, hipStream_t s, const ConvLstmOpts& o = ConvLstmOpts{});
int run_conv3x3s2(const float* x, int cin, int ldx, const float* w, const float* bias, float* out, int cout,
                  int ldo, int relu, int B, int Hin, int Win, hipStream_t s, int accum);
bool conv3x3s2_ln_ok(int cin, int cout, int B, int Hin, int Win);
struct Conv3x3LnOpts { const Enc3Fuse* fuse3; NormKeep keep; };
int run_conv3x3s2_ln(const float* x_raw, int cin, const float* w, const float* bias, float* out, int cout, int ldo, int relu,
                     int B, int Hin, int Win, hipStream_t s, const LnIn& ln, const Conv3x3LnOpts& o = Conv3x3LnOpts{});
struct DeconvOpts {
    int accum;
    LnPartOut ln_out;
    Operand operand;
    const float* wscale_part;
};
int run_deconv3x3s2(const float* x, int cin, int ldx, const float* w, const float* bias, float* out, int cout,
                    int ldo, int relu, int B, int Hin, int Win, hipStream_t s, const DeconvOpts& o = DeconvOpts{});
int run_deconv3x3s2_and_partials(const float* x, int cin, const float* w, const float* bias, float* out, int cout, int ldo, int relu,
                                 int B, int Hin, int Win, hipStream_t s, const float* wt, float* partials, int dbl);
bool deconv3x3s2_ln_ok(int c_ln, int c1, int cout, int B, int Hin, int Win);
struct DeconvLnOpts {
    const float* x1; int c1, ld1;
    LnPartOut ln_out;
    Operand operand;
    const float* wscale_part;
    NormKeep keep;
    const MotionRider* rider;
};
int run_deconv3x3s2_ln(const float* h_raw, int c_ln, const float* w, const float* bias, float* out, int cout, int ldo, int relu,
                       int B, int Hin, int Win, hipStream_t s, const LnIn& ln, const DeconvLnOpts& o = DeconvLnOpts{});
struct ConvS1Opts {
    int accum;
    int wN;
    int dest_zeroed;
    int no_split;
};
int run_conv_s1(const float* x, int cin, int ldx, const float* w, float* out, int cout, int ldo, int ksize, int B, int H, int W,
                hipStream_t s, const ConvS1Opts& o = ConvS1Opts{});
bool conv_s1_splits_k(int cin, int cout, int ldo, int ksize, int B, int H, int W, int wN, int no_split);
bool conv5x5_bf16_splits_k(int cin, int cout, int ldo, int B, int H, int W, Operand form, int no_split);
struct Conv5x5Bf16Opts {
    Operand operand;
    int dest_zeroed;
    const float* ascale_part;
    const EpSpec* ep;
    int no_split;
};
int run_conv5x5_bf16(const float* x, int cin, int ldx, const unsigned short* wb, float* out, int cout, int ldo, int accum,
                     int B, int H, int W, hipStream_t s, const Conv5x5Bf16Opts& o);
struct LayerNormOpts {
    float* stat_out;
    int fused_nparts;
};
int run_layernorm(const float* x, const float* g, const float* b, float* out, float* partials, int B, int n, int C,
                  int ldo, float eps, int relu, hipStream_t s, const LayerNormOpts& o = LayerNormOpts{});

void lstm_wgrad_geom(WgradDesc& d, int cx, int C, int B, int H, int W);
void conv3x3s2_wgrad_geom(WgradDesc& d, int mode, int cin, int cout, int B, int Hin, int Win);
int run_wgrad(WgradDesc& d, hipStream_t s, Operand form, bool fixed_order = false);
long long conv_backward_part_floats(int mode, int cin, int cout, int B, int Hin, int Win);
bool conv_backward_fixed_order(int mode, int cin, int cout, int B, int Hin, int Win);
long long lstm_wgrad_part_floats(int cx, int C, int B, int H, int W, int slot_ntw, int slot_j);
int lstm_wgrad_reduce(int cx, int C, int has_h, float* part, float* dW, float* db, int B, int H, int W, hipStream_t s, int slot_ntw, int slot_j);

struct ConvLstmBwdArgs {
    const float* x; int cx, ldx; const float* h_prev; int C; const float* w; const float* gates;
    const float* c_old; const float* c_new; const float* dh_a; int lda; const float* dh_b; int ldb;
    float* dc; int dc_valid;
    float* dG; float* wt;
    float* d_in;
    float* dW; float* db;
    int B, H, W;
    int wt_ready;
    Operand operand;
    unsigned short* wt_bf16;
    const SideFork* fork;
    const LnFuse* ln;
    int dx_only;
    float* dg_absmax;
    const EpSpec* ep;
    int det;
};
// ... 26 lines not shown
```

### physical-interaction-video-prediction_amd/csrc/pivp_kernels.h

```cpp
#pragma once
#include "pivp_common.h"
#include "conv_form.h"
#include "wgrad_form.h"

namespace pivp {

enum class Operand : int {
    F32 = 0,
    BF16 = 1,
    BF16X3 = 2,
    BF16X6 = 3,
    FP16X3 = 4
};
constexpr int operand_pieces(Operand o) {
    switch (o) {
        case Operand::F32: case Operand::BF16: return 1;
        case Operand::BF16X3: case Operand::FP16X3: return 2;
        case Operand::BF16X6: return 3;
    }
    return 0;
}
constexpr bool operand_l2_direct(Operand o) { return o == Operand::BF16X6 || o == Operand::FP16X3; }
constexpr bool operand_needs_scale(Operand o) { return o == Operand::FP16X3; }

struct IgemmDesc {
    const float* x0; const float* x1;
    int c0, ld0, c1, ld1;
    int wcin;
    const float* w;
    const float* bias;
    int B, Hin, Win;
    int Hg, Wg, in_step;
    int N, M;
    int wN;
    int nphase;
    int deconv, ksize, pad;
    int bytes0, bytes1, bytesw;
    int out_step, Hout, Wout;
    float* out; int ldo; int relu;
    int accum;
    int ksplit_ok;
    int no_ksplit;
    const float* cstate_in; float* cstate_out; float* hout; int C;
    float* gates_out;
    float* ln_part; int ln_cap; int ln_nparts;
    Operand operand;
    const float* wscale_part;
    const float* in_g; const float* in_b; const float* in_part; int in_np; float in_eps;
    float* in_out; int in_out_ld; float* in_stat_out;
    const float* ep_src; int ep_ld, ep_cols, ep_mode;
    int n_mblk; unsigned fd_mb_mul, fd_mb_sh, fd_hw_mul, fd_hw_sh, fd_w_mul, fd_w_sh, fd_cc_mul, fd_cc_sh;
    const float* f3_w; const float* f3_b; const float* f3_action; const float* f3_state; const float* f3_wcs; const float* f3_bcs;
    float* f3_out; float* f3_state_out; int f3_use_state;
    int rd_mode, rd_blocks, rd_KS, rd_nout;
    const float* rd_partials; const float* rd_bias; const float* rd_w2; const float* rd_b2; float* rd_out; float* rd_vpre;
};

struct SideFork {
    hipStream_t side;
    hipEvent_t ready, done;
};
inline int fork_begin(const SideFork* f, hipStream_t s, hipStream_t* sw) {
    *sw = s;
    if (!f || !f->side) return PIVP_OK;
    if (hipEventRecord(f->ready, s) != hipSuccess || hipStreamWaitEvent(f->side, f->ready, 0) != hipSuccess) return PIVP_ERR_LAUNCH;
    *sw = f->side;
    return PIVP_OK;
}
inline int fork_end(const SideFork* f) {
    if (!f || !f->side) return PIVP_OK;
    return hipEventRecord(f->done, f->side) == hipSuccess ? PIVP_OK : PIVP_ERR_LAUNCH;
}

struct WgradDesc {
    const float* x0; const float* x1;
    int c0, ld0, c1, ld1, cin, wcin;
    const float* dy; int ldy, N;
    float* dw;
    int B, Hx, Wx, Hy, Wy;
    int Hg, Wg, M;
    int deconv, ksize, pad, stride;
    int bytes0, bytes1, bytesy;
    float* db;
    int tcount;
    long long ts_x0, ts_x1, ts_dy;
    float* part;
    int part_overwrite;
    const float* dy_absmax; int dy_absmax_stride;
    Operand operand;
    int form;
    int slot_ntw;
    int slot_j;
};
inline WgradShape wgrad_shape(const WgradDesc& d) {
    return {d.c0, d.ld0, d.c1, d.ld1, d.cin, d.wcin, d.ldy, d.N, d.B, d.Hx, d.Wx, d.Hy, d.Wy, d.Hg, d.Wg, d.M, d.deconv, d.ksize, d.pad, d.stride,
            !(d.ts_x0 % 16 || d.ts_x1 % 16 || d.ts_dy % 16)};
}
inline WgradLaunch wgrad_launch(const WgradDesc& d, bool with_part) {
    return wgrad_launch(wgrad_shape(d), (int)d.operand, d.tcount, d.form, d.slot_ntw, d.slot_j, with_part, pivp_cu_count());
}
int igemm_wgrad_check(const WgradDesc& d);
int igemm_wgrad(const WgradDesc& d, const WgradLaunch& L, hipStream_t s);
int igemm_wgrad_reduce(const WgradDesc& d, hipStream_t s);
int wgrad3x3s2(const WgradDesc& d, const WgradLaunch& L, hipStream_t s);
int wgrad3x3s2_reduce(const WgradDesc& d, const WgradLaunch& L, hipStream_t s);
int wgrad5x5p(const WgradDesc& d, const WgradLaunch& L, hipStream_t s);
int wgrad5x5p_reduce(const WgradDesc& d, const WgradLaunch& L, hipStream_t s);
int wgrad5x5p_partition(const WgradDesc& d, int* geom8, int* segs, int seg_cap, int* nsegs, int* slots, int slot_cap, int* nslots);
int wgrad5x5_bf16(const WgradDesc& d, const WgradLaunch& L, hipStream_t s);
int repack_transpose(const float* w, float* wt, int taps, int cin, int N, int flip, hipStream_t s);
struct WeightPrepJob { int kind; const float* src; void* dst; int p0, p1, p2, p3; };
constexpr int WEIGHT_PREP_MAX = 16;
int weight_prep_batch(const WeightPrepJob* jobs, int n, hipStream_t s);

int igemm_lstm(const IgemmDesc& d, hipStream_t stream, int variant = 0, int* ln_nparts = nullptr);
int igemm_conv(const IgemmDesc& d, hipStream_t stream, int* ln_nparts = nullptr);
int igemm_conv_ksplit(const IgemmDesc& d);
int igemm_validate(const IgemmDesc& d, bool lstm);
int igemm_small(const IgemmDesc& d, hipStream_t stream, int* ln_nparts = nullptr);
bool igemm_in_ln_ok(const IgemmDesc& d);
bool deconv_tile_ok(const IgemmDesc& d);
int deconv_tile(const IgemmDesc& d, hipStream_t stream, int* ln_nparts = nullptr);
int absmax_partials(const float* w, long n, float* tail, hipStream_t stream);
size_t lstm_bf16_weight_elems(int wcin, int N);
int pack_lstm_bf16(const float* w, unsigned short* wb, int wcin, int N, hipStream_t s, Operand form, int Np = 0, int plain = 0);
int conv5x5_bf16_rows(int N);
int conv5x5_bf16_ksplit(const IgemmDesc& d, Operand form);
// ... 160 lines not shown
```

### physical-interaction-video-prediction_amd/csrc/plan.h

```cpp
#pragma once
#include <string.h>
#include <string>
#include <vector>

#include "../../include/pivp_hip.h"
#include "../../include/pivp_loss.h"
#include "../../include/pivp_input_grad.h"
#include "../../include/pivp_state.h"
#include "../../include/pivp_state_grad.h"
#include "pivp_host.h"

#pragma GCC visibility push(hidden)
namespace pivp {

struct MapSize { int H, W; };
inline MapSize level_map(const pivp_config_t& c, int level) { return {c.height / level, c.width / level}; }
struct LstmSpec { const char* name; int cx; int C; int level; };
inline const LstmSpec kLstm[7] = {
    {"lstm1", 32, 32, 2}, {"lstm2", 32, 32, 2}, {"lstm3", 32, 64, 4}, {"lstm4", 64, 64, 4},
    {"lstm5", 64, 128, 8}, {"lstm6", 128, 64, 4}, {"lstm7", 96, 32, 2}};
inline MapSize lstm_map(const pivp_config_t& c, int i) { return level_map(c, kLstm[i].level); }
static_assert(STATE_SEGMENTS == PIVP_STATE_SEGMENTS && STATE_SEGMENTS == 2 * 7, "c and h of the seven cells");
inline long long state_seg_floats(const pivp_config_t& c, int g) { const MapSize m = lstm_map(c, g / 2); return (long long)m.H * m.W * kLstm[g / 2].C; }
inline size_t state_seg_offset(const pivp_config_t& c, int g) {
// ... 21 lines not shown
    Operand precision;
    bool packs() const { return precision != Operand::F32; }
    Operand dgrad(int H, int W, int B) const { return operand_l2_direct(precision) && !packed_tiles_serve(H, W, B) ? Operand::F32 : precision; }
    Operand wgrad(int H, int W, int B) const { return precision == Operand::BF16X3 ? Operand::F32 : dgrad(H, W, B); }
    bool wgrad_batches() const { return precision == Operand::BF16 || operand_l2_direct(precision); }
    Operand deconv(bool has_wabs) const { return precision == Operand::BF16X6 || (operand_needs_scale(precision) && !has_wabs) ? Operand::F32 : precision; }
    Operand enc_dgrad() const { return precision == Operand::BF16 ? Operand::BF16 : Operand::F32; }
};

struct ParamInfo { std::string name; long long numel; const float* ptr; float* grad; int group; };

inline int ln_partial_cap(int HW) {
    const int a = ln_stats_slices(64 * HW), b = (HW / 4 / 32 + 1) * 2 * 4;
    return a > b ? a : b;
}

constexpr int DET_SLOT_J = 64;

struct Slab {
    size_t cat7, n1, n2, cat6, n3, n4, e2, e3, n5, e4, e5, e6;
    size_t h[7], c[7];
    size_t e0raw, e6raw;
    size_t gates[7];
    size_t lnstat;
    size_t logits, enc7, layer0, kerns, vpre, theta;
    size_t prevsel;
};

struct Grads {
    size_t cat7, n2, n4, n5, e6;
    size_t e0raw[2], dv[2];
    size_t cat6, e2, e6raw, cat6_sz, e2_sz, e6raw_sz;
    size_t din[7], din_sz[7], dc[7];
    size_t dG[7], go, dmk, dz, dkpart, dstate, lnpart;
    size_t wt_lstm[7], wt_enc[7];
    size_t ln_ppart[9], ln_ppart_floats;
    size_t wg_part[5], wg_part_floats;
    size_t wtb_lstm[7];
    size_t dg_absmax;
    size_t lstm_part[7], det_heads, det_dv, det_enc3, det_enc0, det_stp, det_stp_acc;
};

struct LastRollout {
    int steps;
    bool sched;
    bool predict;
    bool carried;
    const float* state_in;
    bool state_lost;
};

enum class MotionHead { None, Rider, InHead, Separate };
enum class Output { FrameHead, Separate };
struct StepForm {
    bool keep;
    bool norm_inside[9];
    bool enc3_in_enc2;
    bool enc4_partials;
    MotionHead motion;
    Output output;
};

struct StepProfile {
    bool on = false; std::vector<hipEvent_t> ev; std::vector<int> layer; size_t used = 0;
    bool room() const { return used + 2 <= ev.size(); }
    void begin(hipStream_t s) { if (room()) (void)hipEventRecord(ev[used], s); }
    void end(int tag, hipStream_t s) { if (room()) { (void)hipEventRecord(ev[used + 1], s); layer[used / 2] = tag; used += 2; } }
};

}
#pragma GCC visibility pop

struct pivp_plan {
    pivp_config_t cfg;
    std::vector<pivp::ParamInfo> params;
    int i_enc_w[7], i_enc_b[7], i_lstm_w[7], i_lstm_b[7];
    int i_ln_g[9], i_ln_b[9];
    int i_masks_w, i_masks_b, i_cs_w, i_cs_b, i_enc7_w, i_enc7_b;
    int i_head_w, i_head_b, i_head2_w, i_head2_b;
    int H2, W2, H4, W4, H8, W8, NP, NE, K5;
    pivp::Modes mode{pivp::Operand::F32};
    int det = 0;
    int opt[PIVP_OPT_COUNT] = {1, 1, 1, 1, 0};
    pivp::StepForm form = {};
    int wg_cap = 1;
    int eg_cap = 1;
    float* ws; long long ws_floats;
    int nslabs;
    std::vector<pivp::Slab> slabs;
    pivp::Grads g;
    bool has_grads;
    size_t o_zero, o_lnpart, o_lnpart2, o_linpart, o_masks, o_losspart;
    size_t o_wabs[2];
    size_t o_wbf16[7];
    int loss_nparts;
    int pack_cache = 0, packs_valid = 0;
    int main_prio = -1;
    pivp_grad_group_cb grad_cb = nullptr; void* grad_cb_user = nullptr;
    bool group_join = true;
    const float* frame_seed = nullptr;
    float* in_dact = nullptr; float* in_dstate0 = nullptr;
    int sweep_mode = 3;
    const float* state_in = nullptr; float* state_out = nullptr; int observed = 0;
    int sg_enable = 0; const float* sg_seed = nullptr; float* sg_dstate_in = nullptr;
    pivp::LastRollout last = {};
    pivp::StepProfile prof;
    pivp::SideLane lane;
    ~pivp_plan() {
        lane.sync();
        for (hipEvent_t e : prof.ev) (void)hipEventDestroy(e);
        lane.destroy();
    }
};

#pragma GCC visibility push(hidden)
namespace pivp {

inline const float* P(const pivp_plan* p, int idx) { return p->params[idx].ptr; }
inline float* G(const pivp_plan* p, int idx) { return p->params[idx].grad; }

inline bool frame_size_ok(const pivp_config_t& c) { return c.height >= 16 && c.width >= 16 && c.height % 8 == 0 && c.width % 8 == 0; }
inline bool plan_serves_forward(const pivp_config_t& c) {
    return frame_size_ok(c) && composite_serves(c.height, c.width, c.num_masks, c.model_type) &&
           (c.model_type != PIVP_MODEL_CDNA || cdna_kernels_serves(c.num_masks));
}
inline bool plan_serves_backward(const pivp_config_t& c, bool det) {
    return plan_serves_forward(c) && composite_bwd_serves(c.model_type, c.height, c.width, c.num_masks, det);
}

inline StepForm step_form(const pivp_plan& p) {
    const pivp_config_t& c = p.cfg;
    const int B = c.batch, H = c.height, W = c.width;
    const bool train = c.keep_activations != 0, fold_opt = p.opt[PIVP_OPT_LN_FOLD_TRAIN] || !train;
    const Modes& md = p.mode;
    StepForm f = {};
    f.keep = train;
    f.norm_inside[1] = !train && convlstm_ln_in_ok(md.precision, 32, 32, 32, B, p.H2, p.W2) && (long)B * (p.H2 / 8) * (p.W2 / 16) >= 128;
    f.norm_inside[3] = !train && convlstm_ln_in_ok(md.precision, 64, 64, 64, B, p.H4, p.W4) && (long)B * (p.H4 / 8) * (p.W4 / 16) >= 64;
    f.norm_inside[2] = fold_opt && conv3x3s2_ln_ok(32, 32, B, p.H2, p.W2);
    f.norm_inside[4] = fold_opt && conv3x3s2_ln_ok(64, 64, B, p.H4, p.W4);
    f.enc3_in_enc2 = !train && f.norm_inside[4] && p.opt[PIVP_OPT_FUSE_ENC3] && (p.H8 * p.W8) % 32 == 0 &&
                     c.action_dim == 5 && c.state_dim == 5;
    auto fold_small = [](long long floats) { return floats * 4 <= 6LL << 20; };
    f.norm_inside[6] = fold_small((long long)B * 64 * p.H4 * p.W4) && deconv3x3s2_ln_ok(64, 32, 96, B, p.H4, p.W4);
    f.norm_inside[7] = fold_small((long long)B * 32 * p.H2 * p.W2) && deconv3x3s2_ln_ok(32, 32, 64, B, p.H2, p.W2);
    f.norm_inside[8] = (H * W) % 64 == 0;
    const bool fh = frame_head_pays(c.model_type, B, H, W, c.num_masks);
    const bool fh_fin = fh && c.model_type != PIVP_MODEL_DNA && frame_head_finishes(p.K5);
    f.output = fh ? Output::FrameHead : Output::Separate;
    f.enc4_partials = fh_fin && md.deconv(false) == Operand::F32;
    f.motion = c.model_type == PIVP_MODEL_DNA ? MotionHead::None
             : !fh_fin ? MotionHead::Separate
             : f.norm_inside[6] && p.opt[PIVP_OPT_FINISH_RIDER] ? MotionHead::Rider : MotionHead::InHead;
    return f;
}

void plan_layout(pivp_plan* p);
size_t state_bytes(const pivp_config_t& c);
bool ranges_overlap(const void* a, const void* b, size_t bytes);
const float* step_input(const pivp_plan* plan, int t, const float* images, const unsigned char* gt_select, const float* gen_images, size_t fr, int ctx = 0);
int state_grad_gather(const pivp_config_t& c, const float* const dc[7], const float* const din[7], float* d_state_in, hipStream_t s);
int state_grad_scatter(const pivp_config_t& c, const float* d_state_out, float* const dc[7], hipStream_t s);

#define RC(call) do { int rc_ = (call); if (rc_ != PIVP_OK) return rc_; } while (0)

}
// ... 2 lines not shown
```

### physical-interaction-video-prediction_amd/csrc/plan_forward.hip

```cpp
#include "plan.h"

using namespace pivp;

namespace {

struct StepIn { int t; const float* prev; const float* action; const float* state_prev; float* gen_out; float* state_out; };

struct Rollout {
    const pivp_plan& p; hipStream_t s; int ctx; const float* state_in; StepProfile* prof;
    bool masks_every_step = false;
    const pivp_config_t& c = p.cfg; const StepForm& f = p.form; const Modes& md = p.mode;
    float* const ws = p.ws; float* const lnpA = ws + p.o_lnpart; float* const lnpB = ws + p.o_lnpart2;
    const int B = c.batch, H = c.height, W = c.width;
    const float eps = c.ln_eps;
    const int ln_cap = ln_partial_cap(H * W);
    const int n2 = 32 * p.H2 * p.W2, n4 = 64 * p.H4 * p.W4, n8 = 128 * p.H8 * p.W8;
    int t = 0; const Slab* S = nullptr; const Slab* Sp = nullptr;
    float* lnp = nullptr; int np = 0;
    bool enc3_done = false;
    bool partials_done = false;
    MotionHead motion = MotionHead::None;

    const float* hp(int i) const { return Sp ? ws + Sp->h[i] : state_in ? state_in + state_seg_offset(c, 2 * i + 1) : nullptr; }
    const float* cp(int i) const { return Sp ? ws + Sp->c[i] : state_in ? state_in + state_seg_offset(c, 2 * i) : ws + p.o_zero; }
    float* other(float* q) const { return q == lnpA ? lnpB : lnpA; }
    int lstm(int i, const float* x, int ldx, const LnIn* ln_in = nullptr, float* part_out = nullptr) {
        if (prof) prof->begin(s);
        const MapSize m = lstm_map(c, i);
        ConvLstmOpts o{};
        if (f.keep) o.gates_out = ws + S->gates[i];
        o.ln_out.part = part_out ? part_out : lnp; o.ln_out.cap = ln_cap; o.ln_out.nparts = &np;
        if (md.packs()) { o.w_bf16 = reinterpret_cast<const unsigned short*>(ws + p.o_wbf16[i]); o.operand = md.precision; }
        o.ln_in = ln_in;
        int rc = run_convlstm(x, kLstm[i].cx, ldx, hp(i), kLstm[i].C, P(&p, p.i_lstm_w[i]), P(&p, p.i_lstm_b[i]),
                              cp(i), ws + S->c[i], ws + S->h[i], B, m.H, m.W, s, o);
        if (prof) prof->end(i + (hp(i) ? 0 : 8), s);
        return rc;
    }
    float* stat(int j) const { return ws + S->lnstat + (size_t)j * B * 2; }
    int ln(int j, const float* x, float* out, int n, int C, int ldo, int relu) {
        LayerNormOpts o{};
        o.stat_out = stat(j); o.fused_nparts = np;
        return run_layernorm(x, P(&p, p.i_ln_g[j]), P(&p, p.i_ln_b[j]), out, lnp, B, n, C, ldo, eps, relu, s, o);
    }
    LnIn norm_in(int j) const { return LnIn{P(&p, p.i_ln_g[j]), P(&p, p.i_ln_b[j]), lnp, np, eps}; }
    NormKeep keep(int j, float* out, int ld) const { return NormKeep{out, ld, stat(j)}; }
    int lstm_behind_norm(int i, size_t normed, int n) {
        const int C = kLstm[i].cx;
        const float* raw = ws + S->h[i - 1];
        if (f.norm_inside[i] && np > 0) {
            const LnIn li = norm_in(i);
            float* q = other(lnp);
            RC(lstm(i, raw, C, &li, q));
            lnp = q;
            return PIVP_OK;
        }
        RC(ln(i, raw, ws + normed, n, C, C, 0));
        return lstm(i, ws + normed, C);
    }
    int enc_behind_norm(int e, int j, size_t normed, int n, int C, float* out, int ldo, int Hin, int Win, const Enc3Fuse* f3) {
        const float* raw = ws + S->h[j - 1];
        if (f.norm_inside[j] && np > 0) {
            Conv3x3LnOpts o{};
            if (f.keep) o.keep = keep(j, ws + normed, C);
            else o.fuse3 = f3;
            return run_conv3x3s2_ln(raw, C, P(&p, p.i_enc_w[e]), P(&p, p.i_enc_b[e]), out, C, ldo, 1, B, Hin, Win, s, norm_in(j), o);
        }
        RC(ln(j, raw, ws + normed, n, C, C, 0));
        return run_conv3x3s2(ws + normed, C, C, P(&p, p.i_enc_w[e]), P(&p, p.i_enc_b[e]), out, C, ldo, 1, B, Hin, Win, s, 0);
    }
    float* motion_out() const { return ws + (c.model_type == PIVP_MODEL_STP ? S->theta : S->kerns); }
    int motion_dbl() const { return c.model_type == PIVP_MODEL_STP ? 1 : 0; }
    int motion_separate() {
        if (c.model_type == PIVP_MODEL_CDNA)
            return cdna_kernels(ws + S->n5, P(&p, p.i_head_w), P(&p, p.i_head_b), ws + p.o_linpart, ws + S->kerns, B, p.K5, c.num_masks, s, ws + S->vpre);
        return stp_params(ws + S->n5, P(&p, p.i_head_w), P(&p, p.i_head_b), P(&p, p.i_head2_w), P(&p, p.i_head2_b), ws + p.o_linpart,
                          ws + S->theta, B, p.K5, s, ws + S->vpre);
    }
    int linear_partials() {
        if (partials_done) return PIVP_OK;
        partials_done = true;
        return motion_partials(ws + S->n5, P(&p, p.i_head_w), ws + p.o_linpart, B, p.K5, motion_dbl(), s);
    }

    int encoder(const StepIn& in);
    int bottleneck(const StepIn& in);
    int decoder();
    int head(const StepIn& in);
    int step(const StepIn& in) {
        t = in.t;
        S = &p.slabs[t % p.nslabs]; Sp = t > 0 ? &p.slabs[(t - 1) % p.nslabs] : nullptr;
        lnp = lnpA; np = 0;
        enc3_done = partials_done = false;
        motion = f.motion;
        RC(encoder(in));
        RC(bottleneck(in));
        RC(decoder());
        return head(in);
    }
};

int Rollout::encoder(const StepIn& in) {
    RC(conv_enc0(in.prev, P(&p, p.i_enc_w[0]), P(&p, p.i_enc_b[0]), ws + S->e0raw, B, H, W, s, lnp, ln_cap, &np));
    RC(ln(0, ws + S->e0raw, ws + S->cat7 + 32, n2, 32, 64, 1));
    RC(lstm(0, ws + S->cat7 + 32, 64));
    RC(lstm_behind_norm(1, S->n1, n2));
    RC(enc_behind_norm(1, 2, S->n2, n2, 32, ws + S->cat6 + 64, 96, p.H2, p.W2, nullptr));
    RC(lstm(2, ws + S->cat6 + 64, 96));
    RC(lstm_behind_norm(3, S->n3, n4));
    Enc3Fuse f3;
    memset(&f3, 0, sizeof(f3));
    if (f.enc3_in_enc2 && np > 0) {
        f3.w3 = P(&p, p.i_enc_w[3]); f3.b3 = P(&p, p.i_enc_b[3]); f3.action = in.action; f3.state = in.state_prev; f3.wcs = P(&p, p.i_cs_w); f3.bcs = P(&p, p.i_cs_b);
        f3.e3 = ws + S->e3; f3.state_out = in.state_out; f3.use_state = c.use_state;
        enc3_done = true;
    }
// ... 232 lines not shown
```

### physical-interaction-video-prediction_amd/csrc/plan_setup.hip

```cpp
#include "plan.h"

using namespace pivp;

static int grad_group_of(const std::string& n) {
    auto starts = [&](const char* p) { return n.rfind(p, 0) == 0; };
    if (starts("masks/") || starts("model/") || starts("norm_enc6/") || starts("enc6/")) return 0;
    if (starts("hidden7/") || starts("lstm7/")) return 1;
    if (starts("enc5/") || starts("hidden6/") || starts("lstm6/")) return 2;
    if (starts("enc4/") || starts("hidden5/") || starts("lstm5/")) return 3;
    if (starts("enc3/") || starts("current_state/") || starts("enc2/") || starts("hidden4/") || starts("lstm4/") ||
        starts("hidden3/") || starts("lstm3/")) return 4;
    return 5;
}

constexpr size_t ENC_RING_BYTES_MAX = (size_t)2 << 30;
constexpr int WG_BATCH_MAX = 8;

static int wg_cap_of(int T, const Modes& m, int e ) {
    const int want = e ? e : m.precision == Operand::BF16 ? WG_BATCH_MAX : m.wgrad_batches() ? 2 : 1;
    int cap = T - 2 < 1 ? 1 : (T - 2 > WG_BATCH_MAX ? WG_BATCH_MAX : T - 2);
    if (want < cap) cap = want < 1 ? 1 : want;
    return cap;
}
void pivp::plan_layout(pivp_plan* p) {
// ... 154 lines not shown

extern "C" void pivp_plan_destroy(pivp_plan_t* plan) { delete plan; }
extern "C" int pivp_param_count(const pivp_plan_t* plan) { return plan ? (int)plan->params.size() : PIVP_ERR_BADARG; }
extern "C" const char* pivp_param_name(const pivp_plan_t* plan, int idx) {
    if (!plan || idx < 0 || idx >= (int)plan->params.size()) return nullptr;
    return plan->params[idx].name.c_str();
}
extern "C" long long pivp_param_numel(const pivp_plan_t* plan, int idx) {
    if (!plan || idx < 0 || idx >= (int)plan->params.size()) return PIVP_ERR_BADARG;
    return plan->params[idx].numel;
}
extern "C" int pivp_plan_set_param(pivp_plan_t* plan, int idx, const float* dptr) {
    if (!plan || idx < 0 || idx >= (int)plan->params.size() || !dptr) return PIVP_ERR_BADARG;
    plan->params[idx].ptr = dptr;
    plan->packs_valid = 0;
    return PIVP_OK;
}
extern "C" int pivp_param_group(const pivp_plan_t* plan, int idx) {
    if (!plan || idx < 0 || idx >= (int)plan->params.size()) return PIVP_ERR_BADARG;
    return plan->params[idx].group;
}
extern "C" int pivp_param_group_by_name(const char* name) { return name ? grad_group_of(name) : PIVP_ERR_BADARG; }
extern "C" int pivp_plan_set_grad_callback(pivp_plan_t* plan, pivp_grad_group_cb cb, void* user) {
    if (!plan) return PIVP_ERR_BADARG;
    plan->grad_cb = cb; plan->grad_cb_user = user;
    return PIVP_OK;
}
extern "C" int pivp_plan_set_grad(pivp_plan_t* plan, int idx, float* dptr) {
    if (!plan || idx < 0 || idx >= (int)plan->params.size() || !dptr) return PIVP_ERR_BADARG;
    plan->params[idx].grad = dptr;
    return PIVP_OK;
}
static bool det_supported(const pivp_plan* p, Operand precision);
extern "C" int pivp_plan_set_precision(pivp_plan_t* plan, int precision_code) {
    if (!plan || precision_code < PIVP_PRECISION_F32 || precision_code > PIVP_PRECISION_FP16X3) return PIVP_ERR_BADARG;
    const Operand precision = (Operand)precision_code;
    if (plan->det && !det_supported(plan, precision)) return PIVP_ERR_BADARG;
    if (precision == Operand::BF16 || precision == Operand::BF16X3) {
        for (int i = 0; i < 7; ++i) {
            const MapSize m = lstm_map(plan->cfg, i);
            IgemmDesc d;
            memset(&d, 0, sizeof(d));
            d.ksize = 5; d.pad = 2; d.in_step = 1; d.C = kLstm[i].C; d.c0 = kLstm[i].cx; d.c1 = kLstm[i].C;
            d.ld0 = 4; d.ld1 = 4; d.B = plan->cfg.batch; d.Hin = m.H; d.Win = m.W;
            if (!convlstm_bf16_ok(d)) return PIVP_ERR_BADARG;
        }
    }
    const Modes cand{precision};
    if (plan->ws && plan->has_grads && wg_cap_of(plan->cfg.seq_len, cand, plan->opt[PIVP_OPT_WGRAD_BATCH]) > plan->wg_cap) return PIVP_ERR_STATE;
    plan->mode = cand;
    plan->packs_valid = 0;
    if (!plan->ws) plan_layout(plan);
    else plan->form = step_form(*plan);
    return PIVP_OK;
}
static bool det_supported(const pivp_plan* p, Operand precision) {
    if (operand_l2_direct(precision)) return false;
    const int B = p->cfg.batch;
    for (int i = 0; i < 7; ++i) {
        const MapSize m = lstm_map(p->cfg, i);
        if (lstm_wgrad_part_floats(kLstm[i].cx, kLstm[i].C, B, m.H, m.W, 0, DET_SLOT_J) <= 0) return false;
    }
    for (const EncSpec& E : kEnc) {
        const MapSize m = level_map(p->cfg, E.level);
        if (!conv_backward_fixed_order(E.mode, E.c, E.c, B, m.H, m.W)) return false;
    }
    return true;
}
extern "C" int pivp_plan_set_deterministic(pivp_plan_t* plan, int on) {
    if (!plan) return PIVP_ERR_BADARG;
    const int want = on ? 1 : 0;
    if (want == plan->det) return PIVP_OK;
    if (want && !det_supported(plan, plan->mode.precision)) return PIVP_ERR_BADARG;
    if (plan->ws) {
        if (want && plan->has_grads && plan->g.det_heads == 0) return PIVP_ERR_STATE;
        plan->det = want;
        return PIVP_OK;
    }
    plan->det = want;
    plan_layout(plan);
    return PIVP_OK;
}
extern "C" int pivp_plan_get_deterministic(const pivp_plan_t* plan) { return plan ? plan->det : PIVP_ERR_BADARG; }
extern "C" int pivp_plan_set_option(pivp_plan_t* plan, int option, int value) {
    if (!plan || option < 0 || option >= PIVP_OPT_COUNT) return PIVP_ERR_BADARG;
    if (value < 0 || value > (option == PIVP_OPT_WGRAD_BATCH ? WG_BATCH_MAX : 1)) return PIVP_ERR_BADARG;
    if (plan->ws) return PIVP_ERR_STATE;
    plan->opt[option] = value;
    plan_layout(plan);
    return PIVP_OK;
}
extern "C" int pivp_plan_get_option(const pivp_plan_t* plan, int option) {
    return plan && option >= 0 && option < PIVP_OPT_COUNT ? plan->opt[option] : PIVP_ERR_BADARG;
}

extern "C" int pivp_plan_set_frame_grad(pivp_plan_t* plan, const float* seed) {
    if (!plan || (reinterpret_cast<uintptr_t>(seed) & 3)) return PIVP_ERR_BADARG;
    plan->frame_seed = seed;
    return PIVP_OK;
}
extern "C" int pivp_plan_set_input_grad(pivp_plan_t* plan, float* dactions, float* dstate0) {
    if (!plan || ((reinterpret_cast<uintptr_t>(dactions) | reinterpret_cast<uintptr_t>(dstate0)) & 3)) return PIVP_ERR_BADARG;
    plan->in_dact = dactions; plan->in_dstate0 = dstate0;
    return PIVP_OK;
}
extern "C" int pivp_state_layout(const pivp_config_t* cfg, long long seg_floats_per_sample[PIVP_STATE_SEGMENTS], long long* floats_per_sample) {
    if (!cfg || !frame_size_ok(*cfg)) return PIVP_ERR_BADARG;
    long long total = 0;
    for (int g = 0; g < PIVP_STATE_SEGMENTS; ++g) {
        const long long n = state_seg_floats(*cfg, g);
        if (seg_floats_per_sample) seg_floats_per_sample[g] = n;
        total += n;
    }
    if (floats_per_sample) *floats_per_sample = total;
    return PIVP_OK;
}
extern "C" int pivp_plan_set_rollout_state(pivp_plan_t* plan, const float* state_in, float* state_out, int observed) {
    if (!plan || ((reinterpret_cast<uintptr_t>(state_in) | reinterpret_cast<uintptr_t>(state_out)) & 15)) return PIVP_ERR_BADARG;
    if (observed < 0 || observed > plan->cfg.seq_len - 1) return PIVP_ERR_BADARG;
    plan->state_in = state_in; plan->state_out = state_out; plan->observed = observed;
    return PIVP_OK;
}
extern "C" int pivp_plan_get_rollout_state(const pivp_plan_t* plan, const float** state_in, float** state_out, int* observed) {
    if (!plan) return PIVP_ERR_BADARG;
    if (state_in) *state_in = plan->state_in;
    if (state_out) *state_out = plan->state_out;
    if (observed) *observed = plan->observed;
    return PIVP_OK;
}
extern "C" int pivp_state_copy(const pivp_config_t* cfg, const float* src, int B_src, float* dst, int B_dst, const int* index, void* stream) {
    if (!cfg || !src || !dst || B_src < 1 || B_dst < 1 || (!index && B_src != B_dst)) return PIVP_ERR_BADARG;
    if (!frame_size_ok(*cfg)) return PIVP_ERR_BADARG;
    if ((reinterpret_cast<uintptr_t>(src) | reinterpret_cast<uintptr_t>(dst) | reinterpret_cast<uintptr_t>(index)) & 3) return PIVP_ERR_BADARG;
    StateSeg seg[STATE_SEGMENTS];
    long long at = 0;
    for (int g = 0; g < STATE_SEGMENTS; ++g) {
        const long long n = state_seg_floats(*cfg, g);
        seg[g] = StateSeg{src + at * B_src, dst + at * B_dst, n};
        at += n;
    }
    return state_copy(seg, index, B_dst, (hipStream_t)stream);
}
size_t pivp::state_bytes(const pivp_config_t& c) { return (state_seg_offset(c, STATE_SEGMENTS - 1) + (size_t)state_seg_floats(c, STATE_SEGMENTS - 1) * c.batch) * 4; }
bool pivp::ranges_overlap(const void* a, const void* b, size_t bytes) {
    const uintptr_t x = reinterpret_cast<uintptr_t>(a), y = reinterpret_cast<uintptr_t>(b);
    return a && b && x < y + bytes && y < x + bytes;
}
extern "C" int pivp_plan_set_state_grad(pivp_plan_t* plan, int enable, const float* d_state_out, float* d_state_in) {
    if (!plan || (enable != 0 && enable != 1)) return PIVP_ERR_BADARG;
    if ((reinterpret_cast<uintptr_t>(d_state_out) | reinterpret_cast<uintptr_t>(d_state_in)) & 15) return PIVP_ERR_BADARG;
    if (d_state_in && !enable) return PIVP_ERR_BADARG;
    const size_t bytes = state_bytes(plan->cfg);
    if (ranges_overlap(d_state_out, d_state_in, bytes)) return PIVP_ERR_BADARG;
    if (plan->last.carried && ranges_overlap(d_state_in, plan->last.state_in, bytes)) return PIVP_ERR_BADARG;
    plan->sg_enable = enable; plan->sg_seed = d_state_out; plan->sg_dstate_in = d_state_in;
    return PIVP_OK;
}
extern "C" int pivp_plan_get_state_grad(const pivp_plan_t* plan, int* enable, const float** d_state_out, float** d_state_in) {
    if (!plan) return PIVP_ERR_BADARG;
    if (enable) *enable = plan->sg_enable;
    if (d_state_out) *d_state_out = plan->sg_seed;
    if (d_state_in) *d_state_in = plan->sg_dstate_in;
    return PIVP_OK;
}
extern "C" int pivp_plan_set_sweep_mode(pivp_plan_t* plan, int flags) {
    if (!plan || flags < 0 || flags > (PIVP_SWEEP_PARAMS | PIVP_SWEEP_BUILTIN_LOSS)) return PIVP_ERR_BADARG;
    plan->sweep_mode = flags;
    return PIVP_OK;
}
extern "C" int pivp_plan_get_sweep_mode(const pivp_plan_t* plan) { return plan ? plan->sweep_mode : PIVP_ERR_BADARG; }
extern "C" int pivp_plan_set_pack_cache(pivp_plan_t* plan, int on) {
    if (!plan) return PIVP_ERR_BADARG;
    plan->pack_cache = on ? 1 : 0; plan->packs_valid = 0;
    return PIVP_OK;
}
extern "C" int pivp_plan_params_changed(pivp_plan_t* plan) {
// ... 109 lines not shown
```

### physical-interaction-video-prediction_amd/model.py

```python
from __future__ import annotations

import contextlib
import ctypes
import math
import os
import re
from collections import OrderedDict

import numpy as np
import torch

from . import _lib
from . import checkpoint as ckpt
from .state import RecurrentState


class _Config(object):
    train = True


config = _Config()


@contextlib.contextmanager
# ... 1 lines not shown
    old = getattr(config, name)
    setattr(config, name, value)
    try:
        yield
    finally:
        setattr(config, name, old)


LSTM_SIZES = OrderedDict(lstm1=(32, 32), lstm2=(32, 32), lstm3=(32, 64), lstm4=(64, 64),
                         lstm5=(64, 128), lstm6=(128, 64), lstm7=(96, 32))


MAX_INPUT_DIM = 16


def check_input_dim(name, value):
    if isinstance(value, bool) or not isinstance(value, (int, np.integer)) or not 1 <= value <= MAX_INPUT_DIM:
        raise ValueError('%s must be an integer 1 .. %d, not %r' % (name, MAX_INPUT_DIM, value))
    return int(value)


def reference_param_shapes(num_masks, model_type, use_state, height, width, action_dim=5, state_dim=5):
    smear = action_dim + state_dim
    h2, w2, h4, w4, h8, w8 = height // 2, width // 2, height // 4, width // 4, height // 8, width // 8
    s = OrderedDict()
    s['enc0/W'] = (32, 3, 5, 5); s['enc0/b'] = (32,)
    s['enc1/W'] = (32, 32, 3, 3); s['enc1/b'] = (32,)
    s['enc2/W'] = (64, 64, 3, 3); s['enc2/b'] = (64,)
    s['enc3/W'] = (64, 64 + (smear if use_state else 0), 1, 1); s['enc3/b'] = (64,)
    s['enc4/W'] = (128, 128, 3, 3); s['enc4/b'] = (128,)
    s['enc5/W'] = (96, 96, 3, 3); s['enc5/b'] = (96,)
    s['enc6/W'] = (64, 64, 3, 3); s['enc6/b'] = (64,)
    for name, (cx, c) in LSTM_SIZES.items():
        s[name + '/conv/W'] = (4 * c, cx + c, 5, 5)
        s[name + '/conv/b'] = (4 * c,)
    ln = OrderedDict(norm_enc0=32 * h2 * w2, hidden1=32 * h2 * w2, hidden2=32 * h2 * w2, hidden3=64 * h4 * w4,
                     hidden4=64 * h4 * w4, hidden5=128 * h8 * w8, hidden6=64 * h4 * w4, hidden7=32 * h2 * w2,
                     norm_enc6=64 * height * width)
    for name, n in ln.items():
        s[name + '/norm/gamma'] = (n,)
        s[name + '/norm/beta'] = (n,)
    s['masks/W'] = (64, num_masks + 1, 1, 1); s['masks/b'] = (num_masks + 1,)
    s['current_state/W'] = (state_dim, smear); s['current_state/b'] = (state_dim,)
    if model_type == 'CDNA':
        s['model/enc7/W'] = (64, 3, 1, 1); s['model/enc7/b'] = (3,)
        s['model/cdna_kerns/W'] = (25 * num_masks, 128 * h8 * w8); s['model/cdna_kerns/b'] = (25 * num_masks,)
    elif model_type == 'STP':
        s['model/enc7/W'] = (64, 3, 1, 1); s['model/enc7/b'] = (3,)
        s['model/stp_input/W'] = (100, 128 * h8 * w8); s['model/stp_input/b'] = (100,)
        s['model/identity_params/W'] = (6, 100); s['model/identity_params/b'] = (6,)
    else:
        s['model/enc7/W'] = (64, 25, 1, 1); s['model/enc7/b'] = (25,)
    return s


def default_init(shapes, rng=None):
    rng = np.random if rng is None else rng
    out = OrderedDict()
    for key, shape in shapes.items():
        if key.endswith('/W'):
            fan_in = shape[1] if len(shape) == 2 else shape[1] * shape[2] * shape[3]
            out[key] = (rng.standard_normal(shape) * math.sqrt(1.0 / fan_in)).astype(np.float32)
        elif key.endswith('/gamma'):
            out[key] = np.ones(shape, np.float32)
        else:
            out[key] = np.zeros(shape, np.float32)
    return out


def scheduled_sampling_masks(batch_size, seq_len, context_frames, k, iter_num, rng=None):
    rng = np.random if rng is None else rng
    ngt = int(np.int32(np.round(np.float32(batch_size) * (k / (k + np.exp(iter_num / k))))))
    mask = np.zeros((seq_len - 1, batch_size), np.uint8)
    for t in range(seq_len - 1):
        if t > context_frames - 1:
            idx = np.arange(int(batch_size))
            rng.shuffle(idx)
            mask[t, idx[:ngt]] = 1
    return mask


PLAN_OPTIONS = OrderedDict(side_stream=(0, 1, 'PIVP_SIDE_STREAM'), finish_rider=(1, 1, 'PIVP_FINISH_RIDER'), fuse_enc3=(2, 1, 'PIVP_FUSE_ENC3'),
                           ln_fold_train=(3, 1, 'PIVP_LN_FOLD_TRAIN'), wgrad_batch=(4, 0, 'PIVP_WGRAD_BATCH'))
WGRAD_BATCH_MAX = 8


def check_plan_options(given):
    unknown = sorted(set(given or ()) - set(PLAN_OPTIONS))
    if unknown:
        raise ValueError('unknown plan option %s (known: %s)' % (', '.join(map(repr, unknown)), ', '.join(PLAN_OPTIONS)))


def resolve_plan_options(given=None, environ=None):
    check_plan_options(given)
    environ = os.environ if environ is None else environ
    out = OrderedDict()
    for key, (_, default, var) in PLAN_OPTIONS.items():
        env = environ.get(var)
        if given is not None and key in given:
            out[key] = int(given[key])
        elif env is None:
            out[key] = default
        elif key == 'wgrad_batch':
            number = re.match(r'\s*[+-]?\d+', env)
            v = int(number.group()) if number else 0
            out[key] = v if v == 0 else min(max(v, 1), WGRAD_BATCH_MAX)
        else:
            out[key] = 0 if env.startswith('0') else 1
    return out


class _Plan(object):
    def __init__(self, lib, cfg):
        self.lib = lib
        self.cfg = cfg
        h = ctypes.c_void_p()
        _lib.check(lib.pivp_plan_create(ctypes.byref(cfg), ctypes.byref(h)), 'pivp_plan_create')
        self.h = h
        self.names = [lib.pivp_param_name(h, i).decode() for i in range(lib.pivp_param_count(h))]
        self.numel = [lib.pivp_param_numel(h, i) for i in range(len(self.names))]
        self.workspace = None

    def __del__(self):
        try:
            if self.h:
                self.lib.pivp_plan_destroy(self.h)
                self.h = None
        except Exception:
            pass


class Model(object):

    DETERMINISTIC_PRECISIONS = ('fp32', 'bf16', 'bf16x3')

    def __init__(self, num_masks, is_cdna=True, is_dna=False, is_stp=False, use_state=True,
                 scheduled_sampling_k=-1, num_frame_before_prediction=2, prefix=None,
                 device='cuda:0', ln_eps=1e-6, stp_border='clamp', keep_activations=False, precision='fp32', main_priority=None,
                 deterministic=False, image_loss=None, plan_options=None, state_backward=False, action_dim=5, state_dim=5,
                 carry_state=False):
        self.action_dim = check_input_dim('action_dim', action_dim)
        self.state_dim = check_input_dim('state_dim', state_dim)
        if is_cdna:
            self.model_type = 'CDNA'
        elif is_stp:
            self.model_type = 'STP'
        elif is_dna:
            self.model_type = 'DNA'
        else:
            raise ValueError("No network specified")
        self.num_masks = num_masks
        self.use_state = use_state
        self.scheduled_sampling_k = scheduled_sampling_k
        self.sampling_rng = None
        self.num_frame_before_prediction = num_frame_before_prediction
        self.prefix = prefix
        self.device = torch.device(device)
        self.ln_eps = float(ln_eps)
        if stp_border not in ('clamp', 'zeros'):
            raise ValueError("stp_border must be 'clamp' or 'zeros'")
        self.stp_border = stp_border
        self.keep_activations = bool(keep_activations)
        if precision not in ('fp32', 'bf16', 'bf16x3', 'bf16x6', 'fp16x3'):
            raise ValueError("precision must be 'fp32', 'bf16', 'bf16x3', 'bf16x6' or 'fp16x3'")
        self.precision = precision
        if not isinstance(deterministic, bool):
            raise ValueError('deterministic must be a bool, not %r' % (deterministic,))
        if deterministic and precision not in self.DETERMINISTIC_PRECISIONS:
            raise ValueError("deterministic=True is not served with precision=%r (only %s)"
                             % (precision, ', '.join(map(repr, self.DETERMINISTIC_PRECISIONS))))
        self.deterministic = deterministic
        if image_loss is not None:
            from .losses import ImageLoss
            if not isinstance(image_loss, ImageLoss):
                raise ValueError('image_loss must be an ImageLoss or None, not %r' % (image_loss,))
        self.image_loss = image_loss
        self._extra_loss = image_loss is not None and not image_loss.is_reference()
        self.loss_terms = None
        self._loss_grad = None
        self.action_grad = None
        self.state_grad = None
# ... 76 lines not shown
            bounds[-1][2] = off
        self._group_ranges = [(a, b) for _, a, b in bounds]
        flat = np.zeros(off, np.float32)
        for key, v in host.items():
            o, n = offsets[key]
            flat[o:o + n] = v
        new_flat = torch.from_numpy(flat).to(self.device)
        if self._flat_params is not None and self._flat_params.numel() == new_flat.numel():
            self._flat_params.copy_(new_flat)
        else:
            self._flat_params = new_flat
            self._flat_grads = None
        self._offsets = offsets
        self._params = OrderedDict((k, self._flat_params[o:o + n]) for k, (o, n) in offsets.items())
        for plan in self._plans.values():
            self._bind(plan)

    def _ensure_grads(self):
        if self._flat_grads is None:
            self._flat_grads = torch.zeros_like(self._flat_params)
            self._grads = OrderedDict((k, self._flat_grads[o:o + n]) for k, (o, n) in self._offsets.items())
            for plan in self._plans.values():
                self._bind(plan)
        return self._flat_grads

    def load_state_dict_reference(self, ref):
        ref = {k: np.asarray(v) for k, v in ref.items()}
        if self._hw is None:
            self._ref_pending = ref
        else:
            self._require_gpu()
            self._upload(ref, self._shapes())

    def state_dict_reference(self):
        if self._params is None:
            if self._ref_pending is not None:
                return OrderedDict(self._ref_pending)
            raise RuntimeError('parameters are lazily sized from the first input (as in the reference); call the model first')
        out = OrderedDict()
        for key, shape in self._shapes().items():
            out[key] = ckpt.from_internal(key, self._params[key].cpu().numpy(), shape)
        return out

    def count_params(self):
        return sum(int(np.prod(s)) for s in self._shapes().values())

    def params_changed(self):
        self._params_epoch = getattr(self, '_params_epoch', 0) + 1

    def broadcast_params(self, src=0, group=None):
        import torch.distributed as dist
        if self._flat_params is None:
            raise RuntimeError('call the model first (parameters are lazily sized)')
        dist.broadcast(self._flat_params, src=src, group=group)
        self.params_changed()

    def _bind(self, plan):
        lib = plan.lib
        for i, (name, n) in enumerate(zip(plan.names, plan.numel)):
            t = self._params[name]
            if t.numel() != n:
                raise ValueError('%s: internal size %d != library size %d' % (name, t.numel(), n))
            _lib.check(lib.pivp_plan_set_param(plan.h, i, t.data_ptr()), 'pivp_plan_set_param(%s)' % name)
            if self._grads is not None:
                _lib.check(lib.pivp_plan_set_grad(plan.h, i, self._grads[name].data_ptr()), 'pivp_plan_set_grad(%s)' % name)

    def _plan_for(self, B, T, H, W, keep_activations=None, observed=None):
        keep = self.keep_activations if keep_activations is None else bool(keep_activations)
        ctx = self.num_frame_before_prediction if observed is None else min(self.num_frame_before_prediction, T - 1)
        key = (B, T, H, W, keep) if ctx == self.num_frame_before_prediction else (B, T, H, W, keep, ctx)
        plan = self._plans.get(key)
        if plan is None:
            lib = self._require_gpu()
            cfg = _lib.PivpConfig(batch=B, seq_len=T, height=H, width=W, num_masks=self.num_masks,
                                  model_type={'CDNA': 0, 'STP': 1, 'DNA': 2}[self.model_type],
                                  use_state=1 if self.use_state else 0,
                                  context_frames=ctx,
                                  keep_activations=1 if keep else 0,
                                  ln_eps=self.ln_eps, stp_zero_border=1 if self.stp_border == 'zeros' else 0,
                                  action_dim=self.action_dim, state_dim=self.state_dim)
            plan = _Plan(lib, cfg)
            self._ensure_params(H, W)
            for name, value in resolve_plan_options(self.plan_options).items():
                opt, default, _ = PLAN_OPTIONS[name]
                if value != default:
                    _lib.check(lib.pivp_plan_set_option(plan.h, opt, value), 'pivp_plan_set_option(%s, %d)' % (name, value))
            _lib.check(lib.pivp_plan_set_pack_cache(plan.h, 1), 'pivp_plan_set_pack_cache')
            if self.main_priority is not None:
                _lib.check(lib.pivp_plan_set_main_priority(plan.h, 1 if self.main_priority else 0), 'pivp_plan_set_main_priority')
            if self.precision != 'fp32':
                _lib.check(lib.pivp_plan_set_precision(plan.h, {'bf16': 1, 'bf16x3': 2, 'bf16x6': 3, 'fp16x3': 4}[self.precision]),
                           'pivp_plan_set_precision(%s)' % self.precision)
            if self.deterministic:
                if lib.pivp_plan_set_deterministic(plan.h, 1) != 0:
                    raise ValueError('deterministic=True is not served for precision=%r, model %s at B=%d, %dx%d'
                                     % (self.precision, self.model_type, B, H, W))
            nbytes = lib.pivp_plan_workspace_bytes(plan.h)
            plan.workspace = torch.empty(nbytes // 4 + 64, dtype=torch.float32, device=self.device)
            base = plan.workspace.data_ptr()
            aligned = (base + 255) // 256 * 256
            _lib.check(lib.pivp_plan_set_workspace(plan.h, aligned, nbytes), 'pivp_plan_set_workspace')
            self._bind(plan)
            self._plans[key] = plan
            self._reset_plan(plan)
        return plan

    def effective_plan_options(self):
        if self._active is None:
            raise RuntimeError('no plan yet: plans are made by the first call')
        lib, h = self._active.lib, self._active.h
        return OrderedDict((name, int(lib.pivp_plan_get_option(h, opt))) for name, (opt, _, _) in PLAN_OPTIONS.items())

    def _stream(self):
        return torch.cuda.current_stream(self.device).cuda_stream

    def _reset_plan(self, plan):
        with torch.cuda.device(self.device):
            _lib.check(plan.lib.pivp_reset_state(plan.h, self._stream()), 'pivp_reset_state')

    def _check_carried_shape(self, B, H, W):
        s = self._state
        if self.carry_state and s is not None and (s.batch, s.hw) != (B, (H, W)):
            raise ValueError('the model carries the recurrent state of batch %d at %dx%d frames, this call has batch %d at %dx%d: reset_state() first'
                             % (s.batch, s.hw[0], s.hw[1], B, H, W))

    @contextlib.contextmanager
    def _carried(self, plan, B, H, W, advance=True, observed=0):
        if not self.carry_state and not observed:
            yield False
            return
        cur = self._state if self.carry_state else None
        out = None
        if self.carry_state and advance:
            if self.state_backward:
                spare = self._spare_state
                fits = spare is not None and spare is not cur and (spare.batch, spare.hw) == (B, (H, W))
                out = spare if fits else RecurrentState.empty(B, (H, W), self.device)
            else:
                out = cur if cur is not None else RecurrentState.empty(B, (H, W), self.device)
        lib = plan.lib
        try:
            _lib.check(lib.pivp_plan_set_rollout_state(plan.h, cur.data.data_ptr() if cur is not None else None,
                                                       out.data.data_ptr() if out is not None else None, int(observed)), 'pivp_plan_set_rollout_state')
            yield cur is not None
            if out is not None:
                if out is not cur and cur is not None:
                    self._spare_state = cur
                elif self._spare_state is out:
                    self._spare_state = None
                self._state = out
        finally:
            lib.pivp_plan_set_rollout_state(plan.h, None, None, 0)

    def recurrent_state(self):
        if not self.carry_state:
            raise RuntimeError('recurrent_state() needs Model(..., carry_state=True): without it no state exists between calls')
        return None if self._state is None else self._state.clone()

    def set_recurrent_state(self, s):
        if not self.carry_state:
            raise RuntimeError('set_recurrent_state() needs Model(..., carry_state=True)')
        if s is None:
            self._state = None
            return
        self._checked_state(s)
        self._state = s.clone()

    def _checked_state(self, s):
        if not isinstance(s, RecurrentState):
            raise ValueError('a RecurrentState (or None) is expected, not %r' % (type(s).__name__,))
        if self._hw is not None and s.hw != self._hw:
            raise ValueError('the model was sized for %dx%d frames, the state is of %dx%d' % (self._hw + s.hw))
        if s.data.device != self.device and not (s.data.is_cuda and self.device.type == 'cuda' and self.device.index is None):
            raise ValueError('the state lives on %s, the model on %s' % (s.data.device, self.device))
        return True

    def _adopt_state(self, s):
        self._checked_state(s)
        self._state = s

    def reset_state(self):
        self._state = None
        self._carried_start = False
        self.loss = 0.0
        self.psnr_all = 0.0
        self._results = None
        self._imagined = False
        self.loss_terms = None
        self._loss_grad = None
        if self._active is not None:
            self._reset_plan(self._active)

    def to_gpu(self, device=None):
        if device is not None:
# ... 390 lines not shown
```

Baseline: 35220 frames/s.

## Add lean first-step ConvLSTM kernel that skips forget gate and cell-state load

On the first rollout step the ConvLSTM has no previous hidden or cell state, so the forget gate contributes nothing. A LEAN template variant of the f32 implicit-GEMM kernel drops the forget-gate weight columns (3 of 4 gate tiles staged in LDS), splits the remaining gate MFMAs across waves by role, and exchanges partial accumulators through LDS afterwards. It also skips the c_in loads. The path is gated by a plan option that is on by default, and it adds an LDS exchange and a role-dependent branch in the K loop.

New measurement: 35510 frames/s (median of 6 runs). Within noise of the previous version (+0.8%).

```diff
diff --git a/include/pivp_hip.h b/include/pivp_hip.h
--- a/include/pivp_hip.h
+++ b/include/pivp_hip.h
@@ -55,6 +55,7 @@
 int pivp_plan_set_deterministic(pivp_plan_t* plan, int on);
 int pivp_plan_get_deterministic(const pivp_plan_t* plan);
 enum { PIVP_OPT_SIDE_STREAM = 0, PIVP_OPT_FINISH_RIDER, PIVP_OPT_FUSE_ENC3, PIVP_OPT_LN_FOLD_TRAIN, PIVP_OPT_WGRAD_BATCH, PIVP_OPT_COUNT };
+enum { PIVP_OPT_FIRST_STEP_LEAN = 16 };
 int pivp_plan_set_option(pivp_plan_t* plan, int option, int value);
 int pivp_plan_get_option(const pivp_plan_t* plan, int option);
 int pivp_plan_set_pack_cache(pivp_plan_t* plan, int on);
@@ -95,6 +96,7 @@
 int pivp_convlstm(const float* x, int cx, int ldx, const float* h_prev, int C, const float* w, const float* bias,
                   const float* c_in, float* c_out, float* h_out, int B, int H, int W, void* stream);
 
+#define PIVP_CONVLSTM_FIRST_STEP 0x100
 int pivp_convlstm_v(const float* x, int cx, int ldx, const float* h_prev, int C, const float* w, const float* bias,
                     const float* c_in, float* c_out, float* h_out, int B, int H, int W, int variant, void* stream);
 
diff --git a/physical-interaction-video-prediction_amd/csrc/igemm_f32.hip b/physical-interaction-video-prediction_amd/csrc/igemm_f32.hip
--- a/physical-interaction-video-prediction_amd/csrc/igemm_f32.hip
+++ b/physical-interaction-video-prediction_amd/csrc/igemm_f32.hip
@@ -19,11 +19,12 @@
 #define F32_STAMP(i)
 #endif
 
-template <int WM, int WN, int NTB, bool LSTM, int KG = 1>
+template <int WM, int WN, int NTB, bool LSTM, int KG = 1, bool LEAN = false>
 __global__ __launch_bounds__(256 * KG, (KG == 1 && LSTM && WM < 4) ? 2 : 1) void igemm_f32_kernel(const IgemmDesc d) {
     F32_STAMP(0);
     PIVP_SET_MAIN_PRIO();
     static_assert(WM * WN == 4, "4 waves");
+    static_assert(!LEAN || (LSTM && WM == 2 && WN == 2 && NTB == 4), "the first-step form serves the 64-row 2 x 2 ConvLSTM tile");
     static_assert(KG == 1 || (KG == 2 && LSTM), "the in-block K split serves the ConvLSTM tile only");
     static_assert(!LSTM || NTB == 4, "ConvLSTM blocks own 4 gates x 32 channels");
     constexpr int BM = 32 * WM;
@@ -33,7 +34,8 @@
     constexpr int GPT = 32 / CPW;
     constexpr int TPW = LSTM ? 4 / GPT : NTB / WN;
     extern __shared__ __attribute__((aligned(16))) float lds_all[];
-    constexpr int A_FLOATS = BM * IG_P, B_FLOATS = BN * IG_P;
+    constexpr int BNS = LEAN ? 96 : BN;
+    constexpr int A_FLOATS = BM * IG_P, B_FLOATS = BNS * IG_P;
     const int gid = KG > 1 ? __builtin_amdgcn_readfirstlane((int)threadIdx.x >> 8) : 0;
     float* const lds = lds_all + gid * 2 * (A_FLOATS + B_FLOATS);
 
@@ -66,7 +68,7 @@
     const int HWg = d.Hg * d.Wg;
 
     constexpr int NA = (BM * 8 + 255) / 256;
-    constexpr int NB = BN * 8 / 256;
+    constexpr int NB = BNS * 8 / 256;
     constexpr unsigned OOB = 0xC0000000u;
     const int cvec = tid & 7;
     const int prow = tid >> 3;
@@ -118,7 +120,8 @@
 #pragma unroll
     for (int j = 0; j < NB; ++j) {
         const int r = prow + 32 * j;
-        const int col = LSTM ? (r / CB) * d.C + nblk * CB + (r % CB) : nblk * BN + r;
+        const int gate = (LEAN && r / CB == 2) ? 3 : r / CB;
+        const int col = LSTM ? gate * d.C + nblk * CB + (r % CB) : nblk * BN + r;
         b_goff[j] = (col * 32 + cvec * 4) * 4;
     }
     const int lds_wa = (prow * IG_P + cvec * 4);
@@ -197,7 +200,8 @@
 #pragma unroll
     for (int t = 0; t < TPW; ++t) {
         int row;
-        if (LSTM) row = (t * GPT + l31 / CPW) * CB + wn * CPW + (l31 % CPW);
+        if (LEAN && t == 1) row = 2 * CB + l31;
+        else if (LSTM) row = (t * GPT + l31 / CPW) * CB + wn * CPW + (l31 % CPW);
         else      row = (wn * TPW + t) * 32 + l31;
         b_off[t] = 2 * A_FLOATS + row * IG_P + 4 * half;
     }
@@ -207,18 +211,20 @@
     constexpr int PRE = NST < 8 ? NST : 0;
     f32x4 fa[2];
     f32x4 fb[2][TPW];
-    auto read_frag0 = [&](int slot) {
+    auto read_frag0 = [&](int slot, auto HEAVY) {
+        constexpr int NT = decltype(HEAVY)::value ? TPW : 1;
         fa[0] = *reinterpret_cast<const f32x4*>(lds + slot * A_FLOATS + a_off);
 #pragma unroll
-        for (int t = 0; t < TPW; ++t) fb[0][t] = *reinterpret_cast<const f32x4*>(lds + slot * B_FLOATS + b_off[t]);
-    };
-    auto chunk = [&](auto LOAD, auto STORE, auto SET, auto PAR, int buf) {
+        for (int t = 0; t < NT; ++t) fb[0][t] = *reinterpret_cast<const f32x4*>(lds + slot * B_FLOATS + b_off[t]);
+    };
+    auto chunk = [&](auto LOAD, auto STORE, auto SET, auto PAR, auto HEAVY, int buf) {
+        constexpr int NT = decltype(HEAVY)::value ? TPW : 1;
         constexpr bool do_load = decltype(LOAD)::value;
         constexpr bool do_store = decltype(STORE)::value;
         using OTHER = std::integral_constant<int, decltype(SET)::value ^ 1>;
         const float* As = lds + buf * A_FLOATS + a_off;
         const float* Bs = lds + buf * B_FLOATS;
-        read_frag0(buf);
+        read_frag0(buf, HEAVY);
         __builtin_amdgcn_sched_barrier(0);
         auto micro = [&](auto Q, auto S2) {
             constexpr int q = decltype(Q)::value, s2 = decltype(S2)::value, step = q * 4 + s2;
@@ -227,11 +233,13 @@
             if constexpr (s2 == 0 && q < 3) {
                 fa[nxt] = *reinterpret_cast<const f32x4*>(As + 8 * (q + 1));
 #pragma unroll
-                for (int t = 0; t < TPW; ++t) fb[nxt][t] = *reinterpret_cast<const f32x4*>(Bs + b_off[t] + 8 * (q + 1));
-            }
-#pragma unroll
-            for (int t = 0; t < TPW; ++t)
-                accs[ci][t] = __builtin_amdgcn_mfma_f32_32x32x2f32(fa[cur][s2], fb[cur][t][s2], accs[ci][t], 0, 0, 0);
+                for (int t = 0; t < NT; ++t) fb[nxt][t] = *reinterpret_cast<const f32x4*>(Bs + b_off[t] + 8 * (q + 1));
+            }
+#pragma unroll
+            for (int t = 0; t < NT; ++t) {
+                f32x16& a = accs[(LEAN && t == 1) ? 0 : ci][t];
+                a = __builtin_amdgcn_mfma_f32_32x32x2f32(fa[cur][s2], fb[cur][t][s2], a, 0, 0, 0);
+            }
             if constexpr (do_load && PRE == 0 && step == 0) stage_begin();
             if constexpr (do_load && PRE > 0 && step == PRE) stage_a();
             if constexpr (do_load && PRE > 0 && step == PRE + 1) stage_b();
@@ -286,14 +294,22 @@
     float bj = 0.f, bi = 0.f, bf = 0.f, bo = 0.f;
     if constexpr (LSTM) {
         const int C = d.C, ch = nblk * CB + wn * CPW + (l31 % CPW), grp = l31 / CPW;
-        bj = d.bias[ch]; bi = d.bias[C + ch]; bf = d.bias[2 * C + ch] + 1.0f; bo = d.bias[3 * C + ch];
-        const __amdgpu_buffer_rsrc_t rsci = __builtin_amdgcn_make_buffer_rsrc(const_cast<float*>(d.cstate_in), 0, d.M * C * 4, 0x00020000);
+        bj = d.bias[ch]; bi = d.bias[C + ch]; bo = d.bias[3 * C + ch];
+        if constexpr (!LEAN) bf = d.bias[2 * C + ch] + 1.0f;
+        const __amdgpu_buffer_rsrc_t rsci = __builtin_amdgcn_make_buffer_rsrc(const_cast<float*>(d.cstate_in), 0, d.cstate_in ? d.M * C * 4 : 0, 0x00020000);
         const int voc = ((m0 + wm * 32 + 4 * half + (GPT > 1 ? grp : 0)) * C + ch) * 4;
 #pragma unroll
         for (int k = 0; k < OWNR; ++k) {
             const int srow = GPT == 1 ? (k & 3) + 8 * (k >> 2) : GPT == 2 ? 2 * (k & 1) + 8 * (k >> 1) : 8 * k;
-            cpre[k] = __builtin_bit_cast(float, __builtin_amdgcn_raw_buffer_load_b32(rsci, voc, srow * C * 4, 0));
-        }
+            if constexpr (LEAN) cpre[k] = 0.f;
+            else cpre[k] = __builtin_bit_cast(float, __builtin_amdgcn_raw_buffer_load_b32(rsci, voc, srow * C * 4, 0));
+        }
+    }
+    constexpr int ROLE_SLOT = 2 * (A_FLOATS + B_FLOATS);
+    int role = wn ^ gid;
+    if constexpr (LEAN && KG == 1) {
+        static_assert((ROLE_SLOT + 1) * 4 <= ig_lds_bytes<WM, NTB, KG>(), "the role slot lies inside the allocation");
+        if (threadIdx.x == 0) reinterpret_cast<int*>(lds_all)[ROLE_SLOT] = (int)__builtin_amdgcn_s_getreg((3 << 11) | 4) & 1;
     }
 
 #pragma unroll
@@ -308,24 +324,48 @@
         if constexpr (PRE > 0) stage_begin();
         __syncthreads();
         F32_STAMP(1);
-        int it = 0;
-        for (; it + 3 < nchunks; it += 2) {
-            chunk(std::true_type{}, std::true_type{}, S0{}, S0{}, 0); sync();
-            chunk(std::true_type{}, std::true_type{}, S1{}, S1{}, 1); sync();
-        }
-        const int rest = nchunks - it;
-        if (rest == 3) {
-            chunk(std::true_type{}, std::true_type{}, S0{}, S0{}, 0); sync();
-            chunk(std::false_type{}, std::true_type{}, S1{}, S1{}, 1); sync();
-            chunk(std::false_type{}, std::false_type{}, S0{}, S0{}, 0);
-        } else if (rest == 2) {
-            chunk(std::false_type{}, std::true_type{}, S0{}, S0{}, 0); sync();
-            chunk(std::false_type{}, std::false_type{}, S0{}, S1{}, 1);
+        auto k_loop = [&](auto R) {
+            using H0 = std::integral_constant<bool, !LEAN || decltype(R)::value == 0>;
+            using H1 = std::integral_constant<bool, !LEAN || decltype(R)::value == 1>;
+            int it = 0;
+            for (; it + 3 < nchunks; it += 2) {
+                chunk(std::true_type{}, std::true_type{}, S0{}, S0{}, H0{}, 0); sync();
+                chunk(std::true_type{}, std::true_type{}, S1{}, S1{}, H1{}, 1); sync();
+            }
+            const int rest = nchunks - it;
+            if (rest == 3) {
+                chunk(std::true_type{}, std::true_type{}, S0{}, S0{}, H0{}, 0); sync();
+                chunk(std::false_type{}, std::true_type{}, S1{}, S1{}, H1{}, 1); sync();
+                chunk(std::false_type{}, std::false_type{}, S0{}, S0{}, H0{}, 0);
+            } else if (rest == 2) {
+                chunk(std::false_type{}, std::true_type{}, S0{}, S0{}, H0{}, 0); sync();
+                chunk(std::false_type{}, std::false_type{}, S0{}, S1{}, H1{}, 1);
+            } else {
+                chunk(std::false_type{}, std::false_type{}, S0{}, S0{}, H0{}, 0);
+            }
+        };
+        if constexpr (LEAN) {
+            if constexpr (KG == 1) role = wn ^ __builtin_amdgcn_readfirstlane(reinterpret_cast<const int*>(lds_all)[ROLE_SLOT]);
+            if (role) k_loop(S1{}); else k_loop(S0{});
         } else {
-            chunk(std::false_type{}, std::false_type{}, S0{}, S0{}, 0);
+            k_loop(S0{});
         }
     }
     F32_STAMP(2);
+    if constexpr (LEAN) {
+        __syncthreads();
+        float* xo = lds;
+#pragma unroll
+        for (int r = 0; r < 16; ++r) xo[(wave * 16 + r) * 64 + lane] = accs[0][1][r];
+        __syncthreads();
+        const int src = (lane & 32) + wn * CPW + (lane & 15);
+        const int w0 = role ? wave ^ 2 : wave, w1 = w0 ^ 2;
+#pragma unroll
+        for (int r = 0; r < 16; ++r) {
+            accs[0][1][r] = xo[(w0 * 16 + r) * 64 + src];
+            accs[1][1][r] = xo[(w1 * 16 + r) * 64 + src];
+        }
+    }
     if constexpr (NACC > 1) {
 #pragma unroll
         for (int t = 0; t < TPW; ++t)
@@ -404,6 +444,7 @@
 #pragma unroll
                 for (int g = 0; g < GPT; ++g) g4[t * GPT + g] = got[g];
             }
+            if constexpr (LEAN) g4[2] = 0.f;
             const int srow = GPT == 1 ? (k & 3) + 8 * (k >> 2) : GPT == 2 ? 2 * (k & 1) + 8 * (k >> 1) : 8 * k;
             const int so = srow * C * 4;
             const LstmCell cell = lstm_cell<GateActF32>(g4, bj, bi, bf, bo, cpre[k]);
@@ -487,14 +528,14 @@
 #endif
 }
 
-template <int WM, int WN, int NTB, bool LSTM, int KG = 1>
+template <int WM, int WN, int NTB, bool LSTM, int KG = 1, bool LEAN = false>
 static int launch_igemm(const IgemmDesc& d, hipStream_t stream, int ksplit = 1, int* ln_nparts = nullptr) {
     constexpr int BM = 32 * WM, BN = 32 * NTB;
     const int n_nblk = LSTM ? (d.C / (8 * NTB)) : (d.N / BN);
     const int mblk = (d.M + BM - 1) / BM;
     constexpr int lds_bytes = ig_lds_bytes<WM, NTB, KG>();
     static PerDeviceOnce once;
-    if (pivp_ensure_dyn_lds(once, reinterpret_cast<const void*>(&igemm_f32_kernel<WM, WN, NTB, LSTM, KG>), lds_bytes) != PIVP_OK) return PIVP_ERR_LAUNCH;
+    if (pivp_ensure_dyn_lds(once, reinterpret_cast<const void*>(&igemm_f32_kernel<WM, WN, NTB, LSTM, KG, LEAN>), lds_bytes) != PIVP_OK) return PIVP_ERR_LAUNCH;
     dim3 grid(mblk * n_nblk, d.nphase, ksplit);
     IgemmDesc dd = d;
     dd.n_mblk = mblk;
@@ -507,7 +548,7 @@
     dd.ln_nparts = (d.ln_part && ksplit == 1 && hwg % BM == 0 && np <= d.ln_cap) ? np : 0;
     if (!dd.ln_nparts) dd.ln_part = nullptr;
     if (ln_nparts) *ln_nparts = dd.ln_nparts;
-    hipLaunchKernelGGL((igemm_f32_kernel<WM, WN, NTB, LSTM, KG>), grid, dim3(256 * KG), lds_bytes, stream, dd);
+    hipLaunchKernelGGL((igemm_f32_kernel<WM, WN, NTB, LSTM, KG, LEAN>), grid, dim3(256 * KG), lds_bytes, stream, dd);
     return PIVP_LAUNCH_STATUS();
 }
 
@@ -521,7 +562,8 @@
     PIVP_CHECK_ARG(d.bytes0 > 0 && d.bytesw > 0 && (d.c1 == 0 || d.bytes1 > 0));
     PIVP_CHECK_ARG(d.wcin >= d.c0 + d.c1 && d.wcin % 32 == 0);
     if (lstm) {
-        PIVP_CHECK_ARG(d.C > 0 && d.C % 32 == 0 && d.N == 4 * d.C && d.bias && d.cstate_in && d.cstate_out && d.hout);
+        PIVP_CHECK_ARG(d.C > 0 && d.C % 32 == 0 && d.N == 4 * d.C && d.bias && (d.cstate_in || d.first_step) && d.cstate_out && d.hout);
+        PIVP_CHECK_ARG(!d.first_step || (d.c1 == 0 && !d.gates_out));
         PIVP_CHECK_ARG(d.nphase == 1 && d.in_step == 1 && d.Hg == d.Hin && d.Wg == d.Win && d.ksize == 5 && d.pad == 2 && !d.deconv);
         PIVP_CHECK_ARG((long long)d.M * d.C * 4 < (1LL << 31));
     } else {
@@ -543,10 +585,11 @@
     }
     switch (variant) {
         case 4:
-            if (((25 * ((d.c0 + d.c1) >> 5)) & 1) == 0) return launch_igemm<2, 2, 4, true, 2>(d, stream, 1, ln_nparts);
-            return launch_igemm<2, 2, 4, true>(d, stream, 1, ln_nparts);
+            if (((25 * ((d.c0 + d.c1) >> 5)) & 1) == 0)
+                return d.first_step ? launch_igemm<2, 2, 4, true, 2, true>(d, stream, 1, ln_nparts) : launch_igemm<2, 2, 4, true, 2>(d, stream, 1, ln_nparts);
+            return d.first_step ? launch_igemm<2, 2, 4, true, 1, true>(d, stream, 1, ln_nparts) : launch_igemm<2, 2, 4, true>(d, stream, 1, ln_nparts);
         case 1: return launch_igemm<4, 1, 4, true>(d, stream, 1, ln_nparts);
-        case 2: return launch_igemm<2, 2, 4, true>(d, stream, 1, ln_nparts);
+        case 2: return d.first_step ? launch_igemm<2, 2, 4, true, 1, true>(d, stream, 1, ln_nparts) : launch_igemm<2, 2, 4, true>(d, stream, 1, ln_nparts);
         case 3: {
             const int ncc = (d.c0 + d.c1) >> 5;
             if (((25 * ncc) & 1) == 0) return launch_igemm<1, 4, 4, true, 2>(d, stream, 1, ln_nparts);
diff --git a/physical-interaction-video-prediction_amd/csrc/pivp_c_api.hip b/physical-interaction-video-prediction_amd/csrc/pivp_c_api.hip
--- a/physical-interaction-video-prediction_amd/csrc/pivp_c_api.hip
+++ b/physical-interaction-video-prediction_amd/csrc/pivp_c_api.hip
@@ -18,6 +18,7 @@
     const LnIn* const ln_in = o.ln_in;
     const bool l2d = operand_l2_direct(o.operand);
     if ((o.w_bf16 != nullptr) != (o.operand != Operand::F32)) return PIVP_ERR_BADARG;
+    if (o.first_step && (h_prev || o.gates_out || o.operand != Operand::F32 || o.ln_in)) return PIVP_ERR_BADARG;
     IgemmDesc d;
     memset(&d, 0, sizeof(d));
     if (ln_in) {
@@ -35,6 +36,7 @@
     d.bytes0 = (int)b0; d.bytes1 = (int)b1; d.bytesw = (int)bw;
     d.out_step = 1; d.Hout = H; d.Wout = W;
     d.cstate_in = c_in; d.cstate_out = c_out; d.hout = h_out; d.C = C; d.gates_out = o.gates_out;
+    d.first_step = o.first_step ? 1 : 0;
     d.ln_part = o.ln_out.part; d.ln_cap = o.ln_out.cap;
     if (l2d && !convlstm_bf16_ok(d)) return w ? igemm_lstm(d, s, 0, o.ln_out.nparts) : PIVP_ERR_BADARG;
     if (o.w_bf16) return convlstm_bf16(d, o.w_bf16, s, o.operand, o.ln_out.nparts, (l2d && o.variant != 16 && o.variant != 32) ? 0 : o.variant);
@@ -423,9 +425,11 @@
 }
 extern "C" int pivp_convlstm_v(const float* x, int cx, int ldx, const float* h_prev, int C, const float* w, const float* bias,
                                const float* c_in, float* c_out, float* h_out, int B, int H, int W, int variant, void* stream) {
-    if (!x || !w || !bias || !c_in || !c_out || !h_out || variant < 0 || variant > 4) return PIVP_ERR_BADARG;
+    const bool first = (variant & PIVP_CONVLSTM_FIRST_STEP) != 0;
+    variant &= ~PIVP_CONVLSTM_FIRST_STEP;
+    if (!x || !w || !bias || (!c_in && !first) || !c_out || !h_out || variant < 0 || variant > 4 || (first && h_prev)) return PIVP_ERR_BADARG;
     ConvLstmOpts o{};
-    o.variant = variant;
+    o.variant = variant; o.first_step = first;
     return run_convlstm(x, cx, ldx, h_prev, C, w, bias, c_in, c_out, h_out, B, H, W, (hipStream_t)stream, o);
 }
 extern "C" int pivp_convlstm_train(const float* x, int cx, int ldx, const float* h_prev, int C, const float* w, const float* bias,
@@ -752,12 +756,14 @@
                                 const float* c_in, float* c_out, float* h_out, const float* gamma, const float* beta,
                                 float* ln_out, int ldo, float* partials, float eps, int B, int H, int W, int variant, int* fused,
                                 void* stream) {
-    if (!x || !w || !bias || !c_in || !c_out || !h_out || !gamma || !beta || !ln_out || !partials || variant < 0 || variant > 4)
+    const bool first = (variant & PIVP_CONVLSTM_FIRST_STEP) != 0;
+    variant &= ~PIVP_CONVLSTM_FIRST_STEP;
+    if (!x || !w || !bias || (!c_in && !first) || !c_out || !h_out || !gamma || !beta || !ln_out || !partials || variant < 0 || variant > 4 || (first && h_prev))
         return PIVP_ERR_BADARG;
     if (C <= 0 || C % 32) return PIVP_ERR_BADARG;
     int np = 0;
     ConvLstmOpts o{};
-    o.variant = variant; o.ln_out.part = partials; o.ln_out.cap = convlstm_ln_cap(H, W, C); o.ln_out.nparts = &np;
+    o.variant = variant; o.first_step = first; o.ln_out.part = partials; o.ln_out.cap = convlstm_ln_cap(H, W, C); o.ln_out.nparts = &np;
     int rc = run_convlstm(x, cx, ldx, h_prev, C, w, bias, c_in, c_out, h_out, B, H, W, (hipStream_t)stream, o);
     if (rc != PIVP_OK) return rc;
     if (fused) *fused = np > 0;
diff --git a/physical-interaction-video-prediction_amd/csrc/pivp_host.h b/physical-interaction-video-prediction_amd/csrc/pivp_host.h
--- a/physical-interaction-video-prediction_amd/csrc/pivp_host.h
+++ b/physical-interaction-video-prediction_amd/csrc/pivp_host.h
@@ -22,6 +22,7 @@
     Operand operand;
     const unsigned short* w_bf16;
     const LnIn* ln_in;
+    bool first_step;
 };
 bool convlstm_ln_in_ok(Operand form, int cx, int ldx, int C, int B, int H, int W);
 int run_convlstm(const float* x, int cx, int ldx, const float* h_prev, int C, const float* w, const float* bias,
diff --git a/physical-interaction-video-prediction_amd/csrc/pivp_kernels.h b/physical-interaction-video-prediction_amd/csrc/pivp_kernels.h
--- a/physical-interaction-video-prediction_amd/csrc/pivp_kernels.h
+++ b/physical-interaction-video-prediction_amd/csrc/pivp_kernels.h
@@ -43,6 +43,7 @@
     int no_ksplit;
     const float* cstate_in; float* cstate_out; float* hout; int C;
     float* gates_out;
+    int first_step;
     float* ln_part; int ln_cap; int ln_nparts;
     Operand operand;
     const float* wscale_part;
diff --git a/physical-interaction-video-prediction_amd/csrc/plan.h b/physical-interaction-video-prediction_amd/csrc/plan.h
--- a/physical-interaction-video-prediction_amd/csrc/plan.h
+++ b/physical-interaction-video-prediction_amd/csrc/plan.h
@@ -127,6 +127,7 @@
     pivp::Modes mode{pivp::Operand::F32};
     int det = 0;
     int opt[PIVP_OPT_COUNT] = {1, 1, 1, 1, 0};
+    int first_step_lean = 1;
     pivp::StepForm form = {};
     int wg_cap = 1;
     int eg_cap = 1;
diff --git a/physical-interaction-video-prediction_amd/csrc/plan_forward.hip b/physical-interaction-video-prediction_amd/csrc/plan_forward.hip
--- a/physical-interaction-video-prediction_amd/csrc/plan_forward.hip
+++ b/physical-interaction-video-prediction_amd/csrc/plan_forward.hip
@@ -32,6 +32,7 @@
         o.ln_out.part = part_out ? part_out : lnp; o.ln_out.cap = ln_cap; o.ln_out.nparts = &np;
         if (md.packs()) { o.w_bf16 = reinterpret_cast<const unsigned short*>(ws + p.o_wbf16[i]); o.operand = md.precision; }
         o.ln_in = ln_in;
+        o.first_step = p.first_step_lean && !hp(i) && !state_in && !f.keep && !md.packs() && !ln_in;
         int rc = run_convlstm(x, kLstm[i].cx, ldx, hp(i), kLstm[i].C, P(&p, p.i_lstm_w[i]), P(&p, p.i_lstm_b[i]),
                               cp(i), ws + S->c[i], ws + S->h[i], B, m.H, m.W, s, o);
         if (prof) prof->end(i + (hp(i) ? 0 : 8), s);
diff --git a/physical-interaction-video-prediction_amd/csrc/plan_setup.hip b/physical-interaction-video-prediction_amd/csrc/plan_setup.hip
--- a/physical-interaction-video-prediction_amd/csrc/plan_setup.hip
+++ b/physical-interaction-video-prediction_amd/csrc/plan_setup.hip
@@ -260,16 +260,23 @@
     return PIVP_OK;
 }
 extern "C" int pivp_plan_get_deterministic(const pivp_plan_t* plan) { return plan ? plan->det : PIVP_ERR_BADARG; }
+static int* opt_slot(pivp_plan_t* plan, int option) {
+    if (!plan) return nullptr;
+    if (option == PIVP_OPT_FIRST_STEP_LEAN) return &plan->first_step_lean;
+    return option >= 0 && option < PIVP_OPT_COUNT ? &plan->opt[option] : nullptr;
+}
 extern "C" int pivp_plan_set_option(pivp_plan_t* plan, int option, int value) {
-    if (!plan || option < 0 || option >= PIVP_OPT_COUNT) return PIVP_ERR_BADARG;
+    int* const slot = opt_slot(plan, option);
+    if (!slot) return PIVP_ERR_BADARG;
     if (value < 0 || value > (option == PIVP_OPT_WGRAD_BATCH ? WG_BATCH_MAX : 1)) return PIVP_ERR_BADARG;
     if (plan->ws) return PIVP_ERR_STATE;
-    plan->opt[option] = value;
+    *slot = value;
     plan_layout(plan);
     return PIVP_OK;
 }
 extern "C" int pivp_plan_get_option(const pivp_plan_t* plan, int option) {
-    return plan && option >= 0 && option < PIVP_OPT_COUNT ? plan->opt[option] : PIVP_ERR_BADARG;
+    const int* const slot = opt_slot(const_cast<pivp_plan_t*>(plan), option);
+    return slot ? *slot : PIVP_ERR_BADARG;
 }
 
 extern "C" int pivp_plan_set_frame_grad(pivp_plan_t* plan, const float* seed) {
diff --git a/physical-interaction-video-prediction_amd/model.py b/physical-interaction-video-prediction_amd/model.py
--- a/physical-interaction-video-prediction_amd/model.py
+++ b/physical-interaction-video-prediction_amd/model.py
@@ -107,21 +107,25 @@
 
 PLAN_OPTIONS = OrderedDict(side_stream=(0, 1, 'PIVP_SIDE_STREAM'), finish_rider=(1, 1, 'PIVP_FINISH_RIDER'), fuse_enc3=(2, 1, 'PIVP_FUSE_ENC3'),
                            ln_fold_train=(3, 1, 'PIVP_LN_FOLD_TRAIN'), wgrad_batch=(4, 0, 'PIVP_WGRAD_BATCH'))
+LATER_PLAN_OPTIONS = OrderedDict(first_step_lean=(16, 1, 'PIVP_FIRST_STEP_LEAN'))
+ALL_PLAN_OPTIONS = OrderedDict(list(PLAN_OPTIONS.items()) + list(LATER_PLAN_OPTIONS.items()))
 WGRAD_BATCH_MAX = 8
 
 
 def check_plan_options(given):
-    unknown = sorted(set(given or ()) - set(PLAN_OPTIONS))
+    unknown = sorted(set(given or ()) - set(ALL_PLAN_OPTIONS))
     if unknown:
-        raise ValueError('unknown plan option %s (known: %s)' % (', '.join(map(repr, unknown)), ', '.join(PLAN_OPTIONS)))
+        raise ValueError('unknown plan option %s (known: %s)' % (', '.join(map(repr, unknown)), ', '.join(ALL_PLAN_OPTIONS)))
 
 
 def resolve_plan_options(given=None, environ=None):
     check_plan_options(given)
     environ = os.environ if environ is None else environ
     out = OrderedDict()
-    for key, (_, default, var) in PLAN_OPTIONS.items():
+    for key, (_, default, var) in ALL_PLAN_OPTIONS.items():
         env = environ.get(var)
+        if key in LATER_PLAN_OPTIONS and env is None and not (given is not None and key in given):
+            continue
         if given is not None and key in given:
             out[key] = int(given[key])
         elif env is None:
@@ -364,7 +368,7 @@
             plan = _Plan(lib, cfg)
             self._ensure_params(H, W)
             for name, value in resolve_plan_options(self.plan_options).items():
-                opt, default, _ = PLAN_OPTIONS[name]
+                opt, default, _ = ALL_PLAN_OPTIONS[name]
                 if value != default:
                     _lib.check(lib.pivp_plan_set_option(plan.h, opt, value), 'pivp_plan_set_option(%s, %d)' % (name, value))
             _lib.check(lib.pivp_plan_set_pack_cache(plan.h, 1), 'pivp_plan_set_pack_cache')
@@ -391,7 +395,7 @@
         if self._active is None:
             raise RuntimeError('no plan yet: plans are made by the first call')
         lib, h = self._active.lib, self._active.h
-        return OrderedDict((name, int(lib.pivp_plan_get_option(h, opt))) for name, (opt, _, _) in PLAN_OPTIONS.items())
+        return OrderedDict((name, int(lib.pivp_plan_get_option(h, opt))) for name, (opt, _, _) in ALL_PLAN_OPTIONS.items())
 
     def _stream(self):
         return torch.cuda.current_stream(self.device).cuda_stream
```
